# tkeskita/smoothMesh

Measured on AMD Instinct MI355X. Metric: mesh-points smoothed/sec/node (100 iters) + achieved HBM GB/s vs roofline, higher is better.
Workload: dtype f64

## Files before the change

smoothmesh_amd/csrc/kernels_boundary.hpp:

```cpp
#pragma once
#include "kernels.hpp"

namespace smgpu {

constexpr uint8_t BF_CORNER = 1, BF_FEATURE = 2, BF_SMOOTHSURF = 4, BF_CONNECTED = 8, BF_SHARP = 16;
constexpr int BND_ERR_NORMAL = 3, BND_ERR_NOHIT = 4, BND_ERR_STRING = 5;

struct BndView {
    int nB;
    const int* pts;
    uint8_t* flags;
    const double* corner;
    const int* inner;
    const int* bfOff; const int* bfVal;
    const uint8_t* ptClass;
    int nFeat;
    const int* featPts; const int* featString; const int* featOfBnd;
    double* featSum; int* featCnt;
    int nTE;
    const double* tePts; const int* teEdges; const int* teString;
    const int* strOff; const int* strEdges;
    int nNodes;
    const float* wideBox;
    const int* wideRef;
    const double* triVerts;
    double distanceTolerance, internalBlend;
};

__device__ __forceinline__ V3 faceAreaOf(const MeshView& m, const double* __restrict__ P, int f) {
    const int b = m.faceOff[f];
    const int n = m.faceOff[f + 1] - b;
    if (n == 3) {
        const V3 p0 = ldv(P, m.facePts[b]), p1 = ldv(P, m.facePts[b + 1]), p2 = ldv(P, m.facePts[b + 2]);
        return 0.5 * cross(p1 - p0, p2 - p0);
    }
    V3 fCentre = ldv(P, m.facePts[b]);
    for (int i = 1; i < n; ++i) fCentre = fCentre + ldv(P, m.facePts[b + i]);
    fCentre = fCentre / double(n);
    V3 sumN = v3(0, 0, 0);
    double sumA = 0.0;
    V3 thisPoint = ldv(P, m.facePts[b]);
    const V3 first = thisPoint;
    for (int i = 0; i < n; ++i) {
        const V3 nextPoint = (i == n - 1) ? first : ldv(P, m.facePts[b + i + 1]);
        const V3 nn = cross(nextPoint - thisPoint, fCentre - thisPoint);
        sumN = sumN + nn;
        sumA += mag(nn);
        thisPoint = nextPoint;
    }
    if (sumA < SMGPU_ROOTVSMALL) return v3(0, 0, 0);
    return 0.5 * sumN;
}

__device__ __forceinline__ void bndNormalsOf(const MeshView& m, const State& s, const BndView& b, int i) {
    if (s.acc->stop) return;
    if (i >= b.nB) return;
    const int p = b.pts[i];
    V3 n = ldv(s.layerNormal, p);
    const int f0 = b.bfOff[i], f1 = b.bfOff[i + 1];
    for (int k = f0; k < f1; ++k) {
        const V3 cSf = faceAreaOf(m, s.ptsCur, b.bfVal[k]);
        n = n - cSf / mag(cSf);
    }
    if (s.sharedSlot && s.sharedSlot[p] >= 0) { stv(s.layerNormal, p, n); return; }
    uint8_t fl = b.flags[i];
    if (f1 > f0) {
        if (mag(n) < 0.1) { n = v3(0, 0, 0); fl |= BF_SHARP; }
        else fl &= (uint8_t)~BF_SHARP;
        b.flags[i] = fl;
    }
    if (n != v3(0, 0, 0)) n = n / mag(n);
    stv(s.layerNormal, p, n);
}
__global__ void __launch_bounds__(kBlock) k_bnd_normals(MeshView m, State s, BndView b) { bndNormalsOf(m, s, b, blockIdx.x * kBlock + threadIdx.x); }

__device__ __forceinline__ void bndNormalsSharedOf(const State& s, const BndView& b, int nShared, const int* sharedLocal, int i) {
    if (s.acc->stop) return;
    if (i >= nShared) return;
    const int bi = s.bndOfShared[i];
    if (bi < 0) return;
    const double* r = s.combL + (size_t)i * s.lStride;
    V3 n = v3(r[0], r[1], r[2]);
    uint8_t fl = b.flags[bi];
    if (r[6] >= 1.0) {
        if (mag(n) < 0.1) { n = v3(0, 0, 0); fl |= BF_SHARP; }
        else fl &= (uint8_t)~BF_SHARP;
        b.flags[bi] = fl;
    }
    if (n != v3(0, 0, 0)) n = n / mag(n);
    stv(s.layerNormal, sharedLocal[i], n);
}
__global__ void __launch_bounds__(kBlock) k_bnd_normals_shared(State s, BndView b, int nShared, const int* sharedLocal) {
    bndNormalsSharedOf(s, b, nShared, sharedLocal, blockIdx.x * kBlock + threadIdx.x);
}
__global__ void __launch_bounds__(kBlock, 2) k_halo_combineAL(int nShared, const int* __restrict__ peer, const double* __restrict__ ownA,
                                                           const double* __restrict__ recvA, double* __restrict__ combA, int nBlocksTwo, int nMulti,
                                                           const int* multiIdx, const int* multiSlots, int nA, State s, BndView b, int bndOn,
                                                           const int* combOff, const int* combSlots, const double* ownL, const double* recvL,
                                                           double* combL, const int* sharedLocal, PushWait pw) {
    pushWait(pw);
    const int bx = (int)blockIdx.x;
    if (bx < nA) { haloCombineA2Of(bx, nShared, peer, ownA, recvA, combA, nBlocksTwo, nMulti, multiIdx, multiSlots, s.ownFold); return; }
    const int i = (bx - nA) * kBlock + (int)threadIdx.x;
    haloCombineLOf(i, nShared, combOff, combSlots, ownL, recvL, combL, s.lStride, s.ownFold);
    if (bndOn) bndNormalsSharedOf(s, b, nShared, sharedLocal, i);
}

__device__ __forceinline__ V3 projectToEdge(const BndView& b, const V3& pt, int e) {
    const V3 a = ldv(b.tePts, b.teEdges[2 * e]), c = ldv(b.tePts, b.teEdges[2 * e + 1]);
    const double edgeLength = mag(c - a);
    const V3 c2pt = pt - a, edgeVec = c - a;
    const double sN = dot(c2pt, edgeVec) / (edgeLength * edgeLength);
    if (sN <= 1e-6) return a;
    if (sN >= (1.0 - 1e-6)) return c;
    return a + sN * edgeVec;
}

__device__ __forceinline__ void bndFeatureOf(const MeshView& m, const State& s, const BndView& b, int j, int lane) {
    if (s.acc->stop) return;
    if (j >= b.nFeat) return;
    const int p = b.featPts[j], str = b.featString[j];
    V3 sum = v3(0, 0, 0);
    int cnt = 0;
    for (int k = m.ppOff[p]; k < m.ppOff[p + 1]; ++k) {
        const int q = m.ppPt[k];
        if (m.pflags[q] & PF_INTERNAL) continue;
        if (b.ptClass[q] & (BF_FEATURE | BF_CORNER)) continue;
        const V3 pt = ldv(s.ptsCur, q);
        double best = SMGPU_GREAT;
        int bestE = 0x7fffffff;
        V3 bestP = v3(SMGPU_GREAT, SMGPU_GREAT, SMGPU_GREAT);
        const int e0 = (str >= 0) ? b.strOff[str] : 0, e1 = (str >= 0) ? b.strOff[str + 1] : b.nTE;
        for (int ke = e0 + lane; ke < e1; ke += 64) {
            const int e = (str >= 0) ? b.strEdges[ke] : ke;
            const V3 pr = projectToEdge(b, pt, e);
            const double d = mag(pr - pt);
            if (d < best) { best = d; bestE = e; bestP = pr; }
        }
        for (int o = 32; o > 0; o >>= 1) {
            const double od = __shfl_xor(best, o, 64);
            const int oe = __shfl_xor(bestE, o, 64);
            const V3 op = v3(__shfl_xor(bestP.x, o, 64), __shfl_xor(bestP.y, o, 64), __shfl_xor(bestP.z, o, 64));
            if (od < best || (od == best && oe < bestE)) { best = od; bestE = oe; bestP = op; }
        }
        if (bestE == 0x7fffffff) { if (lane == 0) s.acc->err = BND_ERR_STRING; continue; }
        sum = sum + bestP;
        ++cnt;
    }
    if (lane == 0) { stv(b.featSum, j, sum); b.featCnt[j] = cnt; }
}
__global__ void __launch_bounds__(64) k_bnd_feature(MeshView m, State s, BndView b) { bndFeatureOf(m, s, b, (int)blockIdx.x, (int)threadIdx.x); }

template <int T, bool ORG>
__global__ void __launch_bounds__(T, (SMGPU_GEOM_WAVES * T) / 256) k_geom_tile_bnd(MeshView m, State s, GeomTileView g, int wantAvg, int writeFaces,
                                                  const int* tileList, int nLaunch, int xcdMap, int deferN, int deferIter, double* deferLocal,
                                                  double* deferHist, BndView b, int nBndBlocks, int nNormalBlocks) {
    const int bx = (int)blockIdx.x;
    if (bx < nBndBlocks) {
        if (bx < nNormalBlocks) bndNormalsOf(m, s, b, bx * T + (int)threadIdx.x);
        else bndFeatureOf(m, s, b, (bx - nNormalBlocks) * (T / 64) + ((int)threadIdx.x >> 6), (int)threadIdx.x & 63);
        return;
    }
    geomTileBody<T, ORG>(m, s, g, wantAvg, writeFaces, tileList, nLaunch, xcdMap, deferN, deferIter, deferLocal, deferHist, bx - nBndBlocks);
}

__device__ __forceinline__ bool triangleIntersection(const double* __restrict__ tv, const V3& orig, const V3& dir, double tol, double& t, V3& pt) {
    const V3 a = v3(tv[0], tv[1], tv[2]), bb = v3(tv[3], tv[4], tv[5]), c = v3(tv[6], tv[7], tv[8]);
    const V3 edge1 = bb - a, edge2 = c - a;
    const V3 pVec = cross(dir, edge2);
    const double det = dot(edge1, pVec);
    if (det > -SMGPU_ROOTVSMALL && det < SMGPU_ROOTVSMALL) return false;
    const double inv_det = 1.0 / det;
    const V3 tVec = orig - a;
    const double u = dot(tVec, pVec) * inv_det;
    if (u < -tol || u > 1.0 + tol) return false;
    const V3 qVec = cross(tVec, edge1);
    const double v = dot(dir, qVec) * inv_det;
    if (v < -tol || u + v > 1.0 + tol) return false;
    t = dot(edge2, qVec) * inv_det;
    if (t < -tol) return false;
    pt = a + u * edge1 + v * edge2;
    return true;
}

constexpr int kBvhStack = 64;

__device__ __forceinline__ bool findLine(const BndView& b, int* __restrict__ stack, const V3& start, const V3& end, V3& hitPoint) {
    const V3 dir = end - start;
    const double tol = 10.0 * 1.0e-15;
    const double o3[3] = {start.x, start.y, start.z}, d3[3] = {dir.x, dir.y, dir.z};
    double inv[3], oinv[3];
    bool flat[3], neg[3];
#pragma unroll
    for (int a = 0; a < 3; ++a) {
        flat[a] = d3[a] == 0.0;
        neg[a] = d3[a] < 0.0;
        inv[a] = flat[a] ? 0.0 : 1.0 / d3[a];
        oinv[a] = -(o3[a] * inv[a]);
    }
    double best = 0.0;
    int bestId = 0x7fffffff;
    double tLimit = 1.0 + 1e-6;
    int sp = 0;
    if (b.nNodes > 0) stack[kBlock * sp++] = 0;
    while (sp > 0) {
        const int item = stack[kBlock * --sp];
        if (item >= 0) {
            const float4* __restrict__ nb = reinterpret_cast<const float4*>(b.wideBox) + 12 * (size_t)item;
            float bx[48];
#pragma unroll
            for (int q = 0; q < 12; ++q) { const float4 v = nb[q]; bx[4 * q] = v.x; bx[4 * q + 1] = v.y; bx[4 * q + 2] = v.z; bx[4 * q + 3] = v.w; }
            const int4* __restrict__ rc = reinterpret_cast<const int4*>(b.wideRef) + 4 * (size_t)item;
            const int4 r0 = rc[0], r1 = rc[1], c0 = rc[2], c1 = rc[3];
            const int ref[8] = {r0.x, r0.y, r0.z, r0.w, r1.x, r1.y, r1.z, r1.w};
            const int cnt[8] = {c0.x, c0.y, c0.z, c0.w, c1.x, c1.y, c1.z, c1.w};
#pragma unroll
            for (int c = 0; c < 8; ++c) {
                const int n = cnt[c];
                double t0 = -1e-6, t1 = tLimit;
                bool touch = n >= 0;
#pragma unroll
                for (int a = 0; a < 3; ++a) {
                    const double lo = (double)bx[8 * a + c], hi = (double)bx[24 + 8 * a + c];
                    if (flat[a]) { touch = touch && !(o3[a] < lo || o3[a] > hi); }
                    else {
                        const double ta = fma(neg[a] ? hi : lo, inv[a], oinv[a]), tb = fma(neg[a] ? lo : hi, inv[a], oinv[a]);
                        t0 = (ta > t0) ? ta : t0;
                        t1 = (tb < t1) ? tb : t1;
                    }
                }
                if (touch && !(t0 > t1) && sp < kBvhStack) stack[kBlock * sp++] = (n == 0) ? ref[c] : -(16 * ref[c] + n) - 1;
            }
        } else {
            const int code = -(item + 1), first = code >> 4, n = code & 15;
            double tv[4][9];
            int ids[4];
#pragma unroll
            for (int k = 0; k < 4; ++k) {
                if (k < n) {
                    const double2* __restrict__ src = reinterpret_cast<const double2*>(b.triVerts) + 5 * (size_t)(first + k);
                    const double2 q0 = src[0], q1 = src[1], q2 = src[2], q3 = src[3], q4 = src[4];
                    tv[k][0] = q0.x; tv[k][1] = q0.y; tv[k][2] = q1.x; tv[k][3] = q1.y; tv[k][4] = q2.x; tv[k][5] = q2.y;
                    tv[k][6] = q3.x; tv[k][7] = q3.y; tv[k][8] = q4.x;
                    ids[k] = (int)__double_as_longlong(q4.y);
                }
            }
#pragma unroll
            for (int k = 0; k < 4; ++k) {
                double t;
                V3 pt;
                if (k >= n || !triangleIntersection(tv[k], start, dir, tol, t, pt)) continue;
                if (!(t <= 1.0)) continue;
                if (bestId == 0x7fffffff || t < best || (t == best && ids[k] < bestId)) { best = t; bestId = ids[k]; hitPoint = pt; }
            }
            if (bestId != 0x7fffffff) tLimit = fmin(tLimit, best + 1e-6 * (1.0 + fabs(best)));
        }
    }
    return bestId != 0x7fffffff;
}

__device__ __forceinline__ V3 findIntersectionPair(const BndView& b, int* __restrict__ stack, const V3& origPoint, const V3& pointNormal, double searchDistance, int role) {
    const V3 undef = v3(SMGPU_GREAT, SMGPU_GREAT, SMGPU_GREAT);
    const V3 endPoint1 = origPoint + pointNormal * searchDistance;
    const V3 endPoint2 = origPoint - pointNormal * searchDistance;
    V3 mine = undef, h;
    if (findLine(b, stack, origPoint, role ? endPoint2 : endPoint1, h)) mine = h;
    const V3 other = v3(__shfl_xor(mine.x, 1, 64), __shfl_xor(mine.y, 1, 64), __shfl_xor(mine.z, 1, 64));
    const V3 hitPoint1 = sel3(role, other, mine), hitPoint2 = sel3(role, mine, other);
    const double distance1 = mag(origPoint - hitPoint1);
    const double distance2 = mag(origPoint - hitPoint2);
    if (distance1 < distance2) return hitPoint1;
    else if (distance2 < distance1) return hitPoint2;
    if (findLine(b, stack, endPoint1, endPoint2, h)) return h;
    return undef;
}

template <bool FINAL>
__global__ void __launch_bounds__(kBlock) k_bnd_fix(MeshView m, State s, Prm prm, BndView b, int partialBase) {
    if (s.acc->stop) return;
    __shared__ int bvhStack[kBvhStack * kBlock];
    const int t = blockIdx.x * kBlock + threadIdx.x;
    const int i = t >> 1, role = t & 1;
    double dist = 0.0;
    int fcount = 0;
    if (i < b.nB) {
        const int p = b.pts[i];
        const uint8_t fl = b.flags[i];
        const V3 cur = ldv(s.ptsCur, p);
        V3 np = ldv(s.prop, p);
        const V3 undef = v3(SMGPU_GREAT, SMGPU_GREAT, SMGPU_GREAT);
        bool frozen = false;
        const int slot = s.sharedSlot ? s.sharedSlot[p] : -1;
        const double* cl = (slot >= 0) ? s.combL + (size_t)slot * s.lStride : nullptr;
        if (fl & BF_CORNER) np = ldv(b.corner, i);
        else if (fl & BF_FEATURE) {
            const int j = b.featOfBnd[i];
            if (cl) np = v3(cl[10], cl[11], cl[12]) / cl[13];
            else np = ldv(b.featSum, j) / double(b.featCnt[j]);
        } else if (fl & BF_SHARP) frozen = true;
        else if (fl & BF_SMOOTHSURF) {
            const V3 pointNormal = ldv(s.layerNormal, p);
            if (pointNormal == v3(0, 0, 0)) s.acc->err = BND_ERR_NORMAL;
            else {
                double searchDistance = b.distanceTolerance;
                V3 surfPoint = undef;
                for (int it = 0; it < 4; ++it) {
                    searchDistance *= (1.0 / 1e-4);
                    surfPoint = findIntersectionPair(b, bvhStack + threadIdx.x, np, pointNormal, searchDistance, role);
                    if (surfPoint != undef) { np = surfPoint; break; }
                }
                if (surfPoint == undef) s.acc->err = BND_ERR_NOHIT;
            }
        }
        if (role == 0) {
        if ((fl & BF_SMOOTHSURF) && (fl & BF_CONNECTED) && b.inner[i] >= 0 && !(fl & (BF_FEATURE | BF_CORNER | BF_SHARP))) {
            const V3 pointNormal = ldv(s.layerNormal, p);
// ... 52 lines not shown
```

smoothmesh_amd/csrc/kernels_tiled.hpp:

```cpp
#pragma once
#include "kernels.hpp"

#ifndef SMGPU_STAGGER
#define SMGPU_STAGGER 0
#endif
__device__ __forceinline__ void staggerFirstRound(int bid, int resident) {
#if SMGPU_STAGGER
    if (bid < resident) {
        const unsigned slot = __builtin_amdgcn_s_getreg((3 << 11) | (0 << 6) | 4) & 15u;
        for (unsigned k = 0; k < slot; ++k) __builtin_amdgcn_s_sleep(SMGPU_STAGGER);
    }
#else
    (void)bid; (void)resident;
#endif
}
#ifndef SMGPU_ABLATE
#define SMGPU_ABLATE 0
#endif
namespace smgpu {

constexpr unsigned kPad = 0xFFFFu;

struct GeomTileView {
    const int* cellOrder; const int* cellBeg; const int* tpOff; const int* tpIds; const int* tfOff; const int* tfIds;
    const int* fvBase; const uint8_t* fvWidth; const uint16_t* faceVerts;
    const int* cfBase; const uint8_t* cfWidth; const uint16_t* cellFaces;
    const uint8_t* tileFlags;
    const int* meta;
    int maxPoints, maxFaces;
};
struct GeomTileMeta { int tpOff, nPts, tfOff, nFaces, fvBase, fvWidth, cellBeg, nCells, cfBase, cfWidth, flags, pad; };
constexpr int kGeomMetaInts = 12;
typedef const __attribute__((address_space(4))) int* const_int_ptr;
__device__ __forceinline__ GeomTileMeta loadTileMeta(const GeomTileView& g, int tile) {
    const_int_ptr p = (const_int_ptr)(g.meta + (size_t)kGeomMetaInts * tile);
    GeomTileMeta t;
    t.tpOff = p[0]; t.nPts = p[1]; t.tfOff = p[2]; t.nFaces = p[3]; t.fvBase = p[4]; t.fvWidth = p[5];
    t.cellBeg = p[6]; t.nCells = p[7]; t.cfBase = p[8]; t.cfWidth = p[9]; t.flags = p[10]; t.pad = 0;
    return t;
}

struct SmoothTileView {
    const int* ptOrder; const int* ptBeg; const int* tcOff; const int* tcIds; const int* tnOff; const int* tnIds;
    const uint16_t* selfLoc;
    const int* pcBase; const uint8_t* pcWidth; const uint16_t* pcEll;
    const int* ppBase; const uint8_t* ppWidth; const uint16_t* ppEll;
    const uint16_t* pairEll;
    const int* pfBase; const uint8_t* pfWidth; const uint16_t* pfEll;
    const int* meta;
    int maxCells, maxPoints, usePairShare;
};

__device__ __forceinline__ SmoothTileView pickView(bool a, const SmoothTileView& x, const SmoothTileView& y) {
    SmoothTileView v;
#define SMGPU_PICK(F) v.F = a ? x.F : y.F;
    SMGPU_PICK(ptOrder) SMGPU_PICK(ptBeg) SMGPU_PICK(tcOff) SMGPU_PICK(tcIds) SMGPU_PICK(tnOff) SMGPU_PICK(tnIds) SMGPU_PICK(selfLoc)
    SMGPU_PICK(pcBase) SMGPU_PICK(pcWidth) SMGPU_PICK(pcEll) SMGPU_PICK(ppBase) SMGPU_PICK(ppWidth) SMGPU_PICK(ppEll) SMGPU_PICK(pairEll)
    SMGPU_PICK(pfBase) SMGPU_PICK(pfWidth) SMGPU_PICK(pfEll) SMGPU_PICK(meta) SMGPU_PICK(maxCells) SMGPU_PICK(maxPoints) SMGPU_PICK(usePairShare)
#undef SMGPU_PICK
    return v;
}

struct SmoothTileMeta { int ptBeg, nPts, tcOff, nCells, tnOff, nNbrs, pcBase, pcWidth, ppBase, ppWidth, pfBase, pfWidth; };
constexpr int kSmoothMetaInts = 12;
__device__ __forceinline__ SmoothTileMeta loadTileMeta(const SmoothTileView& g, int tile) {
    const_int_ptr p = (const_int_ptr)(g.meta + (size_t)kSmoothMetaInts * tile);
    SmoothTileMeta t;
    t.ptBeg = p[0]; t.nPts = p[1]; t.tcOff = p[2]; t.nCells = p[3]; t.tnOff = p[4]; t.nNbrs = p[5];
    t.pcBase = p[6]; t.pcWidth = p[7]; t.ppBase = p[8]; t.ppWidth = p[9]; t.pfBase = p[10]; t.pfWidth = p[11];
    return t;
}

__device__ __forceinline__ int launchTile(int n, int xcdMap, int b = (int)blockIdx.x) {
    if (!xcdMap) return b;
    const int per = (n + 7) >> 3;
    const int i = (b & 7) * per + (b >> 3);
    return i < n ? i : -1;
}
__host__ __device__ inline int tileGrid(int n, int xcdMap) { return xcdMap ? ((n + 7) >> 3) << 3 : n; }

__device__ __forceinline__ V3 ldsv(const double* x, const double* y, const double* z, int i) { return v3(x[i], y[i], z[i]); }

__device__ __forceinline__ void sqrtExact4(double m0, double m1, double m2, double m3, double& a0, double& a1, double& a2, double& a3) {
    const unsigned h0 = (unsigned)__double2hiint(m0), h1 = (unsigned)__double2hiint(m1), h2 = (unsigned)__double2hiint(m2),
                   h3 = (unsigned)__double2hiint(m3);
    const unsigned lo = min(min(h0, h1), min(h2, h3)), hi = max(max(h0, h1), max(h2, h3));
    if (SMGPU_FPEXACT_FAST && __builtin_expect(lo >= ((1023u - 767u) << 20) && hi < (2047u << 20), 1)) {
        a0 = sqrtCore(m0); a1 = sqrtCore(m1); a2 = sqrtCore(m2); a3 = sqrtCore(m3);
    } else {
        a0 = sqrt(m0); a1 = sqrt(m1); a2 = sqrt(m2); a3 = sqrt(m3);
    }
}

#define SMGPU_ELL_ENTRY(J, E, BODY) { const int j = (J); const unsigned e = (E); if (e != kPad) { BODY } }
#define SMGPU_ELL_FOREACH(ROWS, W4, STRIDE, BODY)                         \
    for (int c_ = 0; c_ < (W4); ++c_) {                                   \
        const ushort4 q_ = (ROWS)[(size_t)c_ * (STRIDE)];                 \
        SMGPU_ELL_ENTRY(4 * c_ + 0, q_.x, BODY)                           \
        SMGPU_ELL_ENTRY(4 * c_ + 1, q_.y, BODY)                           \
        SMGPU_ELL_ENTRY(4 * c_ + 2, q_.z, BODY)                           \
        SMGPU_ELL_ENTRY(4 * c_ + 3, q_.w, BODY)                           \
    }

#define SMGPU_ELL_CHUNK(C, Q, BODY)                                       \
    {                                                                     \
        SMGPU_ELL_ENTRY(4 * (C) + 0, (Q).x, BODY)                         \
        SMGPU_ELL_ENTRY(4 * (C) + 1, (Q).y, BODY)                         \
        SMGPU_ELL_ENTRY(4 * (C) + 2, (Q).z, BODY)                         \
        SMGPU_ELL_ENTRY(4 * (C) + 3, (Q).w, BODY)                         \
    }
#define SMGPU_ELL_FOREACH_PRE(Q0, Q1, ROWS, W4, STRIDE, BODY)             \
    {                                                                     \
        if ((W4) > 0) SMGPU_ELL_CHUNK(0, Q0, BODY)                        \
        if ((W4) > 1) SMGPU_ELL_CHUNK(1, Q1, BODY)                        \
        for (int c_ = 2; c_ < (W4); ++c_) {                               \
            const ushort4 q_ = (ROWS)[(size_t)c_ * (STRIDE)];             \
            SMGPU_ELL_CHUNK(c_, q_, BODY)                                 \
        }                                                                 \
    }

template <int T, int ROUNDS, int STRIDE = 1>
__device__ __forceinline__ void stageRecords(const double* __restrict__ src, const int* __restrict__ ids, int n, double* x,
                                             double* y, double* z, int tid) {
    for (int base = 0; base < n; base += T * ROUNDS) {
        int id[ROUNDS];
#pragma unroll
        for (int u = 0; u < ROUNDS; ++u) {
            const int i = base + u * T + tid;
            id[u] = (i < n) ? ids[i] : -1;
        }
        V3 v[ROUNDS];
#pragma unroll
        for (int u = 0; u < ROUNDS; ++u) v[u] = (id[u] >= 0) ? ldv(src, id[u]) : v3(0, 0, 0);
#pragma unroll
        for (int u = 0; u < ROUNDS; ++u) {
            const int i = base + u * T + tid;
            if (id[u] >= 0) { x[STRIDE * i] = v[u].x; y[STRIDE * i] = v[u].y; z[STRIDE * i] = v[u].z; }
        }
    }
}

template <int T, int R1, int R2>
__device__ __forceinline__ void stageRecords2(const double* __restrict__ s1, const int* __restrict__ i1, int n1, double* x1, double* y1,
                                              double* z1, const double* __restrict__ s2, const int* __restrict__ i2, int n2, double* x2,
                                              double* y2, double* z2, int tid) {
    if (n1 > T * R1 || n2 > T * R2) {
        stageRecords<T, R1>(s1, i1, n1, x1, y1, z1, tid);
        stageRecords<T, R2>(s2, i2, n2, x2, y2, z2, tid);
        return;
    }
    int a[R1], b[R2];
#pragma unroll
    for (int u = 0; u < R1; ++u) { const int i = u * T + tid; a[u] = (i < n1) ? i1[i] : -1; }
#pragma unroll
    for (int u = 0; u < R2; ++u) { const int i = u * T + tid; b[u] = (i < n2) ? i2[i] : -1; }
    V3 va[R1], vb[R2];
#pragma unroll
    for (int u = 0; u < R1; ++u) va[u] = (a[u] >= 0) ? ldv(s1, a[u]) : v3(0, 0, 0);
#pragma unroll
    for (int u = 0; u < R2; ++u) vb[u] = (b[u] >= 0) ? ldv(s2, b[u]) : v3(0, 0, 0);
#pragma unroll
    for (int u = 0; u < R1; ++u) { const int i = u * T + tid; if (a[u] >= 0) { x1[i] = va[u].x; y1[i] = va[u].y; z1[i] = va[u].z; } }
#pragma unroll
    for (int u = 0; u < R2; ++u) { const int i = u * T + tid; if (b[u] >= 0) { x2[i] = vb[u].x; y2[i] = vb[u].y; z2[i] = vb[u].z; } }
}

template <int T, int R>
__device__ __forceinline__ void stageRecordsPair(const double* __restrict__ s1, const double* __restrict__ s2, const int* __restrict__ ids,
                                                 int n, double* x1, double* y1, double* z1, double* x2, double* y2, double* z2, int tid) {
    for (int base = 0; base < n; base += T * R) {
        int id[R];
#pragma unroll
        for (int u = 0; u < R; ++u) { const int i = base + u * T + tid; id[u] = (i < n) ? ids[i] : -1; }
        V3 va[R], vb[R];
#pragma unroll
        for (int u = 0; u < R; ++u) { va[u] = (id[u] >= 0) ? ldv(s1, id[u]) : v3(0, 0, 0); vb[u] = (id[u] >= 0) ? ldv(s2, id[u]) : v3(0, 0, 0); }
#pragma unroll
        for (int u = 0; u < R; ++u) {
            const int i = base + u * T + tid;
            if (id[u] >= 0) { x1[i] = va[u].x; y1[i] = va[u].y; z1[i] = va[u].z; x2[i] = vb[u].x; y2[i] = vb[u].y; z2[i] = vb[u].z; }
        }
    }
}

template <int T>
__device__ __forceinline__ void stageRecordsCoh(const double* src, const int* __restrict__ ids, int n, double* x, double* y, double* z, int tid) {
    for (int i = tid; i < n; i += T) { const V3 v = ldvCoh(src, ids[i]); x[i] = v.x; y[i] = v.y; z[i] = v.z; }
}

#ifndef SMGPU_GEOM_AOS
#define SMGPU_GEOM_AOS 1
#endif
constexpr int kGP = SMGPU_GEOM_AOS ? 3 : 1;
#ifndef SMGPU_GEOM_LDS_B64
#define SMGPU_GEOM_LDS_B64 1
#endif
__device__ __forceinline__ V3 ldsg(const double* x, const double* y, const double* z, int i) {
#if SMGPU_GEOM_LDS_B64
    typedef const volatile __attribute__((address_space(3))) double* LdsPtr;
    const LdsPtr vx = (LdsPtr)x, vy = (LdsPtr)y, vz = (LdsPtr)z;
    return v3(vx[i], vy[i], vz[i]);
#else
    return v3(x[i], y[i], z[i]);
#endif
}
#ifndef SMGPU_GEOM_FACE_STRIDE
#define SMGPU_GEOM_FACE_STRIDE 6
#endif
constexpr int kGF = SMGPU_GEOM_AOS ? SMGPU_GEOM_FACE_STRIDE : 1;
struct GeomLds {
    double *px, *py, *pz;
    double *fcx, *fcy, *fcz;
    double *fax, *fay, *faz;
};
__device__ __forceinline__ GeomLds geomLds(double* lds, const GeomTileMeta& tm) {
    GeomLds L;
    if (SMGPU_GEOM_AOS) {
        L.px = lds;                      L.py = L.px + 1;  L.pz = L.px + 2;
        L.fcx = L.px + 3 * tm.nPts;      L.fcy = L.fcx + 1; L.fcz = L.fcx + 2;
        L.fax = L.fcx + 3;               L.fay = L.fcx + 4; L.faz = L.fcx + 5;
        return L;
    }
    L.px = lds;                  L.py = L.px + tm.nPts;    L.pz = L.py + tm.nPts;
    L.fcx = L.pz + tm.nPts;      L.fcy = L.fcx + tm.nFaces; L.fcz = L.fcy + tm.nFaces;
    L.fax = L.fcz + tm.nFaces;   L.fay = L.fax + tm.nFaces; L.faz = L.fay + tm.nFaces;
    return L;
}

template <bool ORG>
__device__ __forceinline__ void geomFace(const State& s, const GeomTileView& g, const GeomLds& L, const GeomTileMeta& tm, int i, unsigned tflags,
                                         int wantAvg, int writeFaces, bool pre = false, ushort4 preQ = make_ushort4(0, 0, 0, 0)) {
    const double *px = L.px, *py = L.py, *pz = L.pz;
    const int b = tm.tfOff;
    const int fw4 = tm.fvWidth >> 2;
    const ushort4* fvTile = reinterpret_cast<const ushort4*>(g.faceVerts + tm.fvBase);
    V3 fCentre, ctr, area;
    if (!ORG && (tflags & 1u)) {
        const ushort4 q = pre ? preQ : fvTile[i];
        const V3 p0 = ldsg(px, py, pz, kGP * (q.x)), p1 = ldsg(px, py, pz, kGP * (q.y)), p2 = ldsg(px, py, pz, kGP * (q.z)), p3 = ldsg(px, py, pz, kGP * (q.w));
        fCentre = divByCount(((p0 + p1) + p2) + p3, 4);
        V3 sumN = v3(0, 0, 0), sumAc = v3(0, 0, 0);
        double sumA = 0.0;
        const V3 n0 = cross(p1 - p0, fCentre - p0), n1 = cross(p2 - p1, fCentre - p1), n2 = cross(p3 - p2, fCentre - p2),
                 n3 = cross(p0 - p3, fCentre - p3);
        double a0, a1, a2, a3;
        sqrtExact4(magSqr(n0), magSqr(n1), magSqr(n2), magSqr(n3), a0, a1, a2, a3);
#define SMGPU_FAN4(THIS, NEXT, NN, A)                                          \
    {                                                                          \
        const V3 c = ((THIS) + (NEXT)) + fCentre;                              \
        sumN = sumN + (NN);                                                    \
        sumA += (A);                                                           \
        sumAc = sumAc + (A) * c;                                               \
    }
        SMGPU_FAN4(p0, p1, n0, a0) SMGPU_FAN4(p1, p2, n1, a1) SMGPU_FAN4(p2, p3, n2, a2) SMGPU_FAN4(p3, p0, n3, a3)
#undef SMGPU_FAN4
        if (sumA < SMGPU_ROOTVSMALL) { ctr = fCentre; area = v3(0, 0, 0); }
        else { ctr = divExact((1.0 / 3.0) * sumAc, sumA); area = 0.5 * sumN; }
    } else {
        const ushort4* row = fvTile + (size_t)i * fw4;
        fCentre = v3(0, 0, 0);
        int n = 0;
        SMGPU_ELL_FOREACH(row, fw4, 1, {
            const V3 p = ldsg(px, py, pz, kGP * (e));
            fCentre = (j == 0) ? p : fCentre + p;
            n = j + 1;
        })
        fCentre = divByCount(fCentre, n);
        if (n == 3) {
            const ushort4 q = row[0];
            const V3 p0 = ldsg(px, py, pz, kGP * (q.x)), p1 = ldsg(px, py, pz, kGP * (q.y)), p2 = ldsg(px, py, pz, kGP * (q.z));
            ctr = (1.0 / 3.0) * ((p0 + p1) + p2);
            area = 0.5 * cross(p1 - p0, p2 - p0);
        } else if (ORG) {
            V3 sumA = v3(0, 0, 0);
            V3 first = v3(0, 0, 0), thisPoint = v3(0, 0, 0);
            SMGPU_ELL_FOREACH(row, fw4, 1, {
                const V3 p = ldsg(px, py, pz, kGP * (e));
                if (j == 0) { first = p; thisPoint = p; }
                else { sumA = sumA + cross(p - thisPoint, fCentre - thisPoint); thisPoint = p; }
            })
            sumA = sumA + cross(first - thisPoint, fCentre - thisPoint);
            const V3 sumAHat = sumA / mag(sumA);
            double sumAn = 0.0;
            V3 sumAnc = v3(0, 0, 0);
#define SMGPU_FAN_ORG(NEXT)                                                    \
    {                                                                          \
        const V3 nextPoint = (NEXT);                                           \
        const V3 a = cross(nextPoint - thisPoint, fCentre - thisPoint);        \
        const V3 c = (thisPoint + nextPoint) + fCentre;                        \
        const double an = dot(a, sumAHat);                                     \
        sumAn += an;                                                           \
        sumAnc = sumAnc + an * c;                                              \
        thisPoint = nextPoint;                                                 \
    }
            SMGPU_ELL_FOREACH(row, fw4, 1, {
                const V3 p = ldsg(px, py, pz, kGP * (e));
                if (j == 0) { first = p; thisPoint = p; }
                else SMGPU_FAN_ORG(p)
            })
            SMGPU_FAN_ORG(first)
#undef SMGPU_FAN_ORG
            if (sumAn > SMGPU_VSMALL) ctr = ((1.0 / 3.0) * sumAnc) / sumAn;
            else ctr = fCentre;
            area = 0.5 * sumA;
        } else {
            V3 sumN = v3(0, 0, 0), sumAc = v3(0, 0, 0);
            double sumA = 0.0;
            V3 first = v3(0, 0, 0), thisPoint = v3(0, 0, 0);
#define SMGPU_FAN(NEXT)                                                        \
    {                                                                          \
        const V3 nextPoint = (NEXT);                                           \
        const V3 c = (thisPoint + nextPoint) + fCentre;                        \
        const V3 nn = cross(nextPoint - thisPoint, fCentre - thisPoint);       \
        const double a = sqrtExact(magSqr(nn));                                \
        sumN = sumN + nn;                                                      \
        sumA += a;                                                             \
        sumAc = sumAc + a * c;                                                 \
        thisPoint = nextPoint;                                                 \
    }
            SMGPU_ELL_FOREACH(row, fw4, 1, {
                const V3 p = ldsg(px, py, pz, kGP * (e));
                if (j == 0) { first = p; thisPoint = p; }
                else SMGPU_FAN(p)
            })
            SMGPU_FAN(first)
#undef SMGPU_FAN
            if (sumA < SMGPU_ROOTVSMALL) { ctr = fCentre; area = v3(0, 0, 0); }
            else { ctr = divExact((1.0 / 3.0) * sumAc, sumA); area = 0.5 * sumN; }
        }
    }
    L.fcx[kGF * i] = ctr.x; L.fcy[kGF * i] = ctr.y; L.fcz[kGF * i] = ctr.z;
    L.fax[kGF * i] = area.x; L.fay[kGF * i] = area.y; L.faz[kGF * i] = area.z;
    if (wantAvg && s.avgPacked) stv(s.fAvg, b + i, fCentre);
    if ((wantAvg && !s.avgPacked) || writeFaces) {
        const int fid = g.tfIds[b + i];
        if (fid < 0) {
            const int f = fid & 0x7fffffff;
            if (wantAvg && !s.avgPacked) stv(s.fAvg, f, fCentre);
            if (writeFaces) { stv(s.fCtr, f, ctr); stv(s.fArea, f, area); }
        }
    }
}

struct GeomCellIn { bool mine; int c; ushort4 qa, qb; };
template <int T>
__device__ __forceinline__ GeomCellIn geomCellLoad(const GeomTileView& g, const GeomTileMeta& tm, int tid, unsigned tflags) {
    GeomCellIn in;
    const int ci = tm.cellBeg + tid;
    in.mine = tid < tm.nCells;
    in.c = 0;
    in.qa = in.qb = make_ushort4(0, 0, 0, 0);
    if (in.mine) {
        in.c = g.cellOrder[ci];
        if ((tflags & 2u)) {
            const ushort4* row = reinterpret_cast<const ushort4*>(g.cellFaces + tm.cfBase) + tid;
            in.qa = row[0]; in.qb = row[T];
        }
    }
    return in;
}
template <int T, bool ORG>
__device__ __forceinline__ void geomCell(const State& s, const GeomTileView& g, const GeomLds& L, const GeomTileMeta& tm, int tid, unsigned tflags, const GeomCellIn& in,
                                         bool coh = false) {
    const double *fcx = L.fcx, *fcy = L.fcy, *fcz = L.fcz, *fax = L.fax, *fay = L.fay, *faz = L.faz;
    if (!in.mine) return;
    const int c = in.c;
    const int cw4 = tm.cfWidth >> 2;
    const ushort4* row = reinterpret_cast<const ushort4*>(g.cellFaces + tm.cfBase) + tid;
    V3 cEst = v3(0, 0, 0), ctr = v3(0, 0, 0);
    double vol = 0.0;
#define SMGPU_PYR(E, FC)                                                                                   \
    {                                                                                                      \
        const V3 fA = ldsg(fax, fay, faz, kGF * ((E) & 0x7fff));                                                   \
         \
        double pyr3Vol = dot(fA, (FC) - cEst);                                                             \
        pyr3Vol = ((E) & 0x8000) ? -pyr3Vol : pyr3Vol;                                                     \
        if (ORG) pyr3Vol = (pyr3Vol > SMGPU_VSMALL) ? pyr3Vol : SMGPU_VSMALL;    \
        const V3 pc = (3.0 / 4.0) * (FC) + (1.0 / 4.0) * cEst;                                             \
        ctr = ctr + pyr3Vol * pc;                                                                          \
        vol += pyr3Vol;                                                                                    \
    }
    if ((tflags & 2u)) {
        const ushort4 qa = in.qa, qb = in.qb;
        const unsigned e0 = qa.x, e1 = qa.y, e2 = qa.z, e3 = qa.w, e4 = qb.x, e5 = qb.y;
        const V3 c0 = ldsg(fcx, fcy, fcz, kGF * (e0 & 0x7fff)), c1 = ldsg(fcx, fcy, fcz, kGF * (e1 & 0x7fff)), c2 = ldsg(fcx, fcy, fcz, kGF * (e2 & 0x7fff)),
                 c3 = ldsg(fcx, fcy, fcz, kGF * (e3 & 0x7fff)), c4 = ldsg(fcx, fcy, fcz, kGF * (e4 & 0x7fff)), c5 = ldsg(fcx, fcy, fcz, kGF * (e5 & 0x7fff));
        cEst = cEst + c0; cEst = cEst + c1; cEst = cEst + c2; cEst = cEst + c3; cEst = cEst + c4; cEst = cEst + c5;
        cEst = divExact(cEst, 6.0);
        SMGPU_PYR(e0, c0) SMGPU_PYR(e1, c1) SMGPU_PYR(e2, c2) SMGPU_PYR(e3, c3) SMGPU_PYR(e4, c4) SMGPU_PYR(e5, c5)
    } else {
        int nFaces = 0;
        SMGPU_ELL_FOREACH(row, cw4, T, {
            cEst = cEst + ldsg(fcx, fcy, fcz, kGF * (e & 0x7fff));
            nFaces = j + 1;
        })
        cEst = divByCount(cEst, nFaces);
        SMGPU_ELL_FOREACH(row, cw4, T, {
            (void)j;
            const V3 fc = ldsg(fcx, fcy, fcz, kGF * (e & 0x7fff));
            SMGPU_PYR(e, fc)
        })
    }
#undef SMGPU_PYR
    if (fabs(vol) > SMGPU_VSMALL) ctr = divExact(ctr, vol);
    else ctr = cEst;
    if (coh) stvCoh(s.cellCtr, c, ctr); else stv(s.cellCtr, c, ctr);
}

#ifndef SMGPU_GEOM_WAVES
#define SMGPU_GEOM_WAVES 5
#endif
template <int T>
__device__ __forceinline__ void geomLoadIds(const GeomTileView& g, const GeomTileMeta& tm, int tid, int (&id)[2]) {
    const int* ids = g.tpIds + tm.tpOff;
#pragma unroll
    for (int u = 0; u < 2; ++u) { const int i = u * T + tid; id[u] = (i < tm.nPts) ? ids[i] : -1; }
}
struct GeomRows { ushort4 fq[2]; GeomCellIn cin; bool preFaces; };
template <int T, bool ORG>
__device__ __forceinline__ GeomRows geomLoadRows(const GeomTileView& g, const GeomTileMeta& tm, int tid) {
    GeomRows r;
    const unsigned tflags = (unsigned)tm.flags;
    r.preFaces = !ORG && (tflags & 1u);
#pragma unroll
    for (int u = 0; u < 2; ++u) {
        const int i = u * T + tid;
        r.fq[u] = (r.preFaces && i < tm.nFaces) ? reinterpret_cast<const ushort4*>(g.faceVerts + tm.fvBase)[i] : make_ushort4(0, 0, 0, 0);
    }
    r.cin = geomCellLoad<T>(g, tm, tid, tflags);
    return r;
}
__device__ __forceinline__ void geomLoadPoints(const State& s, const int (&id)[2], V3 (&v)[2]) {
#pragma unroll
    for (int u = 0; u < 2; ++u) v[u] = (id[u] >= 0) ? ldv(s.ptsCur, id[u]) : v3(0, 0, 0);
}
template <int T>
__device__ __forceinline__ void geomStorePoints(const State& s, const GeomTileView& g, const GeomTileMeta& tm, const GeomLds& L, const int (&id)[2],
                                                const V3 (&v)[2], int tid) {
#pragma unroll
    for (int u = 0; u < 2; ++u) {
        const int i = u * T + tid;
        if (id[u] >= 0) { L.px[kGP * i] = v[u].x; L.py[kGP * i] = v[u].y; L.pz[kGP * i] = v[u].z; }
    }
    if (tm.nPts > 2 * T)
        stageRecords<T, 2, kGP>(s.ptsCur, g.tpIds + tm.tpOff + 2 * T, tm.nPts - 2 * T, L.px + kGP * 2 * T, L.py + kGP * 2 * T, L.pz + kGP * 2 * T, tid);
}
template <int T, bool ORG>
__device__ __forceinline__ void geomFaces(const State& s, const GeomTileView& g, const GeomLds& L, const GeomTileMeta& tm, const GeomRows& r, int tid,
                                          int wantAvg, int writeFaces) {
    const unsigned tflags = (unsigned)tm.flags;
    const int nf = tm.nFaces;
#pragma unroll
    for (int u = 0; u < 2; ++u) {
        const int i = u * T + tid;
        if (i < nf) geomFace<ORG>(s, g, L, tm, i, tflags, wantAvg, writeFaces, r.preFaces, r.fq[u]);
    }
    for (int i = 2 * T + tid; i < nf; i += T) geomFace<ORG>(s, g, L, tm, i, tflags, wantAvg, writeFaces);
}

template <int T, bool ORG>
__device__ __forceinline__ void geomTileBody(const MeshView& m, const State& s, const GeomTileView& g, int wantAvg, int writeFaces, const int* tileList,
                                             int nLaunch, int xcdMap, int deferN, int deferIter, double* deferLocal, double* deferHist, int bid, bool coh = false) {
    const int stopped = s.acc->stop;
    const int li = launchTile(nLaunch, xcdMap, bid);
    if (li < 0) return;
    staggerFirstRound(bid, 256 * 4);
    if (deferN > 0 && bid == 0) { if (stopped) return; finishPartials<T>(s, deferN, deferIter, -1.0, deferLocal, deferHist); __syncthreads(); }
    extern __shared__ double lds[];
    const int tid = threadIdx.x;
    const int tile = tileList ? ((const_int_ptr)tileList)[li] : li;
    const GeomTileMeta tm = loadTileMeta(g, tile);
    const GeomLds L = geomLds(lds, tm);
    int id[2];
    geomLoadIds<T>(g, tm, tid, id);
    const GeomRows r = geomLoadRows<T, ORG>(g, tm, tid);
    V3 v[2];
    geomLoadPoints(s, id, v);
    geomStorePoints<T>(s, g, tm, L, id, v, tid);
    if (stopped) return;
    __syncthreads();
    if (SMGPU_ABLATE & 32) { if (tid < tm.nCells) stv(s.cellCtr, ((const_int_ptr)g.cellOrder)[tm.cellBeg + tid], v3(L.px[tid], 0.0, 0.0)); return; }
    geomFaces<T, ORG>(s, g, L, tm, r, tid, wantAvg, writeFaces);
    __syncthreads();
    if (SMGPU_ABLATE & 64) return;
    geomCell<T, ORG>(s, g, L, tm, tid, (unsigned)tm.flags, r.cin, coh);
}
template <int T, bool ORG>
__global__ void __launch_bounds__(T, (SMGPU_GEOM_WAVES * T) / 256) k_geom_tile(MeshView m, State s, GeomTileView g, int wantAvg, int writeFaces, const int* tileList,
                                                  int nLaunch, int xcdMap, int deferN, int deferIter, double* deferLocal,
                                                  double* deferHist) {
    geomTileBody<T, ORG>(m, s, g, wantAvg, writeFaces, tileList, nLaunch, xcdMap, deferN, deferIter, deferLocal, deferHist, (int)blockIdx.x);
}

struct SmoothLds { double *cx, *cy, *cz, *nx, *ny, *nz; };
__device__ __forceinline__ SmoothLds smoothLds(double* lds, const SmoothTileMeta& tm) {
    SmoothLds L;
    L.cx = lds;                 L.cy = L.cx + tm.nCells;  L.cz = L.cy + tm.nCells;
    L.nx = L.cz + tm.nCells;    L.ny = L.nx + tm.nNbrs;   L.nz = L.ny + tm.nNbrs;
    return L;
}
struct Top3 {
    double l1 = 0, l2 = 0, l3 = 0;
    unsigned w1 = 0xFFFFFFFFu, w2 = 0xFFFFFFFFu, w3 = 0xFFFFFFFFu;
    __device__ __forceinline__ void offer(double len, int j, unsigned e, bool take) {
        const unsigned w = ((unsigned)j << 16) | e;
        const bool b1 = take && (w1 == 0xFFFFFFFFu || len < l1);
        const bool b2 = take && !b1 && (w2 == 0xFFFFFFFFu || len < l2);
        const bool b3 = take && !b1 && !b2 && (w3 == 0xFFFFFFFFu || len < l3);
        const bool b12 = b1 || b2;
        l3 = b12 ? l2 : (b3 ? len : l3);  w3 = b12 ? w2 : (b3 ? w : w3);
        l2 = b1 ? l1 : (b2 ? len : l2);   w2 = b1 ? w1 : (b2 ? w : w2);
        l1 = b1 ? len : l1;               w1 = b1 ? w : w1;
    }
    __device__ __forceinline__ bool has2() const { return w2 != 0xFFFFFFFFu; }
    __device__ __forceinline__ bool has3() const { return w3 != 0xFFFFFFFFu; }
    __device__ __forceinline__ int k1() const { return (int)(w1 >> 16); }
    __device__ __forceinline__ int k2() const { return (int)(w2 >> 16); }
};
struct SmoothRow {
    bool mine; int p, selfL, wn4, wc4, slot;
    int peer, dst0, ndst;
    unsigned fl;
    const ushort4 *ppRow, *pcRow;
    ushort4 pp0, pp1, pc0, pc1;
    ushort4 pe0, pe1;
};
template <int T>
__device__ __forceinline__ unsigned pairBits(const SmoothTileView& g, const SmoothTileMeta& tm, const SmoothRow& R, int tid, int k) {
    if (k < 8) {
        const ushort4 q = (k & 4) ? R.pe1 : R.pe0;
        const unsigned lo = (k & 1) ? q.y : q.x, hi = (k & 1) ? q.w : q.z;
        return (k & 2) ? hi : lo;
    }
    const uint16_t* pe = g.pairEll + tm.ppBase;
    return pe[((size_t)(k >> 2) * T + tid) * 4 + (k & 3)];
}
struct SlotTabs { const int* slot; const int* peer; const int* dst0; const int* ndst; };
template <int T, bool COHC = false, int SLOTS = 1>
__device__ __forceinline__ SmoothRow smoothStage(const MeshView& m, const State& s, const SmoothTileView& g, const SmoothTileMeta& tm,
                                                 const SmoothLds& L, int tid, const SlotTabs& tb = SlotTabs{nullptr, nullptr, nullptr, nullptr}) {
    SmoothRow r;
    r.peer = -1; r.dst0 = -1; r.ndst = 0;
    r.mine = tid < tm.nPts;
    r.wn4 = tm.ppWidth >> 2; r.wc4 = tm.pcWidth >> 2;
    const int lane = r.mine ? tid : 0;
    r.ppRow = reinterpret_cast<const ushort4*>(g.ppEll + tm.ppBase) + tid;
    r.pcRow = reinterpret_cast<const ushort4*>(g.pcEll + tm.pcBase) + tid;
    const bool fast = tm.nCells <= 2 * T && tm.nNbrs <= 3 * T && r.wn4 > 0 && r.wc4 > 0;
    const ushort4 padq = make_ushort4(0xFFFF, 0xFFFF, 0xFFFF, 0xFFFF);
    if (fast) {
        const int* ic = g.tcIds + tm.tcOff;
        const int* in = g.tnIds + tm.tnOff;
        int a[2], b[3];
#pragma unroll
        for (int u = 0; u < 2; ++u) { const int i = u * T + tid; a[u] = (i < tm.nCells) ? ic[i] : -1; }
#pragma unroll
        for (int u = 0; u < 3; ++u) { const int i = u * T + tid; b[u] = (i < tm.nNbrs) ? in[i] : -1; }
        const int pi = tm.ptBeg + lane;
        const int p = g.ptOrder[pi];
        const int selfL = g.selfLoc[pi];
        const ushort4* ppl = reinterpret_cast<const ushort4*>(g.ppEll + tm.ppBase) + lane;
        const ushort4* pcl = reinterpret_cast<const ushort4*>(g.pcEll + tm.pcBase) + lane;
        const ushort4 pp0 = ppl[0], pp1 = ppl[r.wn4 > 1 ? T : 0], pc0 = pcl[0], pc1 = pcl[r.wc4 > 1 ? T : 0];
        const ushort4* pel = reinterpret_cast<const ushort4*>((g.usePairShare ? g.pairEll : g.ppEll) + tm.ppBase) + lane;
        r.pe0 = pel[0]; r.pe1 = pel[r.wn4 > 1 ? T : 0];
        int slot = -1, peer = -1, dst0 = -1, ndst = 0;
        if (SLOTS == 2) { slot = tb.slot[pi]; if (tb.peer) { peer = tb.peer[pi]; dst0 = tb.dst0[pi]; ndst = tb.ndst[pi]; } }
        V3 va[2], vb[3];
#pragma unroll
        for (int u = 0; u < 2; ++u) va[u] = (a[u] >= 0) ? (COHC ? ldvCoh(s.cellCtr, a[u]) : ldv(s.cellCtr, a[u])) : v3(0, 0, 0);
#pragma unroll
        for (int u = 0; u < 3; ++u) vb[u] = (b[u] >= 0) ? ldv(s.ptsCur, b[u]) : v3(0, 0, 0);
        const unsigned fl = m.pflags[p];
        if (SLOTS == 1) slot = s.sharedSlot ? s.sharedSlot[p] : -1;
#pragma unroll
        for (int u = 0; u < 2; ++u) { const int i = u * T + tid; if (a[u] >= 0) { L.cx[i] = va[u].x; L.cy[i] = va[u].y; L.cz[i] = va[u].z; } }
#pragma unroll
        for (int u = 0; u < 3; ++u) { const int i = u * T + tid; if (b[u] >= 0) { L.nx[i] = vb[u].x; L.ny[i] = vb[u].y; L.nz[i] = vb[u].z; } }
        r.p = r.mine ? p : 0; r.selfL = r.mine ? selfL : 0;
        r.fl = fl; r.slot = r.mine ? slot : -1; r.peer = r.mine ? peer : -1; r.dst0 = dst0; r.ndst = r.mine ? ndst : 0;
        r.pp0 = r.mine ? pp0 : padq; r.pp1 = (r.mine && r.wn4 > 1) ? pp1 : padq;
        r.pc0 = r.mine ? pc0 : padq; r.pc1 = (r.mine && r.wc4 > 1) ? pc1 : padq;
        return r;
    }
    r.p = 0; r.selfL = 0; r.fl = 0; r.slot = -1;
    r.pp0 = padq; r.pp1 = padq; r.pc0 = padq; r.pc1 = padq; r.pe0 = padq; r.pe1 = padq;
    if (r.mine) {
        if (g.usePairShare) {
            const ushort4* peRow = reinterpret_cast<const ushort4*>(g.pairEll + tm.ppBase) + tid;
            if (r.wn4 > 0) r.pe0 = peRow[0];
            if (r.wn4 > 1) r.pe1 = peRow[T];
        }
        const int pi = tm.ptBeg + tid;
        r.p = g.ptOrder[pi];
        r.selfL = g.selfLoc[pi];
        if (r.wn4 > 0) r.pp0 = r.ppRow[0];
        if (r.wn4 > 1) r.pp1 = r.ppRow[T];
        if (r.wc4 > 0) r.pc0 = r.pcRow[0];
        if (r.wc4 > 1) r.pc1 = r.pcRow[T];
        r.fl = m.pflags[r.p];
        if (SLOTS == 1) r.slot = s.sharedSlot ? s.sharedSlot[r.p] : -1;
        if (SLOTS == 2) { r.slot = tb.slot[pi]; if (tb.peer) { r.peer = tb.peer[pi]; r.dst0 = tb.dst0[pi]; r.ndst = tb.ndst[pi]; } }
    }
    if (COHC) stageRecordsCoh<T>(s.cellCtr, g.tcIds + tm.tcOff, tm.nCells, L.cx, L.cy, L.cz, tid);
    else stageRecords<T, 2>(s.cellCtr, g.tcIds + tm.tcOff, tm.nCells, L.cx, L.cy, L.cz, tid);
    stageRecords<T, 3>(s.ptsCur, g.tnIds + tm.tnOff, tm.nNbrs, L.nx, L.ny, L.nz, tid);
    return r;
}

template <bool FINAL, int T, int MODE = 0>
__device__ __forceinline__ void smoothPoint(const MeshView& m, const State& s, const Prm& prm, const SmoothTileView& g, const SmoothLds& L,
                                            const SmoothRow& R, const SmoothTileMeta& tm, int tid, double& dist, int& fcount, bool spTile = false) {
    const double *cx = L.cx, *cy = L.cy, *cz = L.cz, *nx = L.nx, *ny = L.ny, *nz = L.nz;
    const bool mine = R.mine;
    const int p = R.p, selfL = R.selfL, wn4 = R.wn4, wc4 = R.wc4;
    const ushort4 *ppRow = R.ppRow, *pcRow = R.pcRow;
    const ushort4 pp0 = R.pp0, pp1 = R.pp1, pc0 = R.pc0, pc1 = R.pc1;
    if ((SMGPU_ABLATE & 16) && !spTile) { if (mine) stv(FINAL ? s.ptsNext : s.prop, p, ldsv(nx, ny, nz, selfL)); return; }
    if (mine && !(MODE == 2 && !spTile && R.slot >= 0)) {
        const unsigned fl = R.fl;
        const bool internal = fl & PF_INTERNAL;
        const V3 cur = ldsv(nx, ny, nz, selfL);
        V3 sum = v3(0, 0, 0), r1, r2, r3;
        double m1 = 0.0, m2 = 0.0, m3 = 0.0;
        int count = 0, hc = 0;
        double shortestCur = SMGPU_GREAT;
        const int slot = (MODE == 1 || (MODE == 2 && !spTile)) ? -1 : R.slot;
        if (slot >= 0) {
            {
                const double* r = s.combA + (size_t)slot * SMGPU_HALO_A_DOUBLES;
                double w[SMGPU_HALO_A_DOUBLES];
#pragma unroll
                for (int q = 0; q < SMGPU_HALO_A_DOUBLES; ++q) w[q] = (MODE == 2 && R.peer < 0) ? ldCoh(r + q) : r[q];
                sum = v3(w[0], w[1], w[2]);
                r1 = v3(w[3], w[4], w[5]); r2 = v3(w[6], w[7], w[8]); r3 = v3(w[9], w[10], w[11]);
                const long long pk = __double_as_longlong(w[12]);
                count = (int)(pk & 0xffffffffll);
                hc = (int)(pk >> 32);
            }
            m1 = mag(r1); m2 = mag(r2); m3 = mag(r3);
            SMGPU_ELL_FOREACH_PRE(pp0, pp1, ppRow, wn4, T, {
                (void)j;
                const double len = mag(cur - ldsv(nx, ny, nz, e & 0x7fff));
                if (len < shortestCur) shortestCur = len;
            })
        } else {
            if (internal || prm.bndOn) {
                if (!(SMGPU_ABLATE & 8))
                SMGPU_ELL_FOREACH_PRE(pc0, pc1, pcRow, wc4, T, {
                    sum = sum + ldsv(cx, cy, cz, (SMGPU_ABLATE & 2) ? 0 : e);
                    count = j + 1;
                })
            }
            Top3 t3;
            SMGPU_ELL_FOREACH_PRE(pp0, pp1, ppRow, wn4, T, {
                const V3 dv_ = cur - ldsv(nx, ny, nz, (SMGPU_ABLATE & 2) ? 0 : (e & 0x7fff));
                const double len = (SMGPU_ABLATE & 1) ? magSqr(dv_) : mag(dv_);
                if (len < shortestCur) shortestCur = len;
                t3.offer(len, j, e, internal || !(e & 0x8000));
            })
            if (!t3.has2()) { s.acc->err = 1; r1 = r2 = r3 = v3(0, 0, 0); }
            else {
                r1 = ldsv(nx, ny, nz, t3.w1 & 0x7fff) - cur;
                r2 = ldsv(nx, ny, nz, t3.w2 & 0x7fff) - cur;
                r3 = !t3.has3() ? v3(SMGPU_GREAT, SMGPU_GREAT, SMGPU_GREAT) : ldsv(nx, ny, nz, t3.w3 & 0x7fff) - cur;
                m1 = t3.l1; m2 = t3.l2; m3 = !t3.has3() ? mag(r3) : t3.l3;
                if (g.usePairShare) {
                    hc = (pairBits<T>(g, tm, R, tid, t3.k1()) >> t3.k2()) & 1;
                } else {
                    const int nb = m.ppOff[p];
                    hc = shareCell(m, m.ppPt[nb + t3.k1()], m.ppPt[nb + t3.k2()]) ? 1 : 0;
                }
            }
        }
        V3 np = cur;
        if (count) np = divByCount(sum, count);
        const double blendFrac = arRatioLen(r1, r2, m1, m2, m3, hc != 0, internal);
        if (blendFrac > 0.0) {
            const V3 aCoords = cur + 0.5 * (r1 + r2);
            np = (1.0 - blendFrac) * np + blendFrac * aCoords;
        }
        {
            const V3 stepDir = np - cur;
            const double len = mag(stepDir);
            const double globalScale = (len > prm.maxStep) ? prm.maxStep / (len * prm.relStepFrac) : 1.0;
            np = cur + (prm.relStepFrac * globalScale) * stepDir;
        }
        if (prm.layersOn) np = layerTreat(s, prm, p, internal, cur, np);
        const bool deferBnd = prm.bndOn && !internal;
        if (prm.bndOn && internal) {
            const V3 stepDir = np - cur;
            const double len = mag(stepDir);
            const double globalScale = (len > prm.maxStep) ? prm.maxStep / (len * prm.relStepFrac) : 1.0;
            np = cur + (prm.relStepFrac * globalScale) * stepDir;
        }
        bool frozen = false;
        {
            double minSqr = __builtin_inf();
            if (!(SMGPU_ABLATE & 4))
            SMGPU_ELL_FOREACH_PRE(pp0, pp1, ppRow, wn4, T, {
                (void)j;
                const double t2 = magSqr(np - ldsv(nx, ny, nz, (SMGPU_ABLATE & 2) ? 0 : (e & 0x7fff)));
                if (t2 < minSqr) minSqr = t2;
            })
            const double rootMin = sqrtExact(minSqr);
            const double shortestNew = (rootMin < SMGPU_GREAT) ? rootMin : SMGPU_GREAT;
            const double shortest = (shortestNew < shortestCur) ? shortestNew : shortestCur;
            if (prm.totalMinFreeze && (shortest < prm.minEdge)) frozen = true;
            else if ((shortestNew < prm.minEdge) && (shortestNew < shortestCur)) frozen = true;
        }
        if (deferBnd) stv(s.prop, p, np);
        else if (FINAL && slot >= 0) {
            if (MODE == 2 && s.ownF) {
                stvCoh(s.prop, p, np);
                __hip_atomic_store(s.ownF + slot, frozen ? 1 : 0, __ATOMIC_RELAXED, __HIP_MEMORY_SCOPE_AGENT);
            } else stv(s.prop, p, np);
            s.frozen[p] = frozen ? 1 : 0;
            if (MODE == 2) {
                const int v = frozen ? 1 : 0;
                if (R.ndst == 1) { if (s.push.slotF) stPeer(s.push.slotF[R.dst0], v); else s.sendF[R.dst0] = v; }
                else
                    for (int k = s.sendOff[slot]; k < s.sendOff[slot + 1]; ++k) {
                        const int sl = s.sendSlots[k];
                        if (s.push.slotF) stPeer(s.push.slotF[sl], v); else s.sendF[sl] = v;
                    }
            } else if (s.inlinePackF)
                for (int k = s.sendOff[slot]; k < s.sendOff[slot + 1]; ++k) s.sendF[s.sendSlots[k]] = frozen ? 1 : 0;
        } else if (FINAL) {
            if (frozen || (!internal && !(fl & PF_SMOOTHSURF))) { np = cur; fcount = 1; }
            dist = mag(np - cur) / prm.maxStep;
            stv(s.ptsNext, p, np);
        } else {
            stv(s.prop, p, np);
            s.frozen[p] = frozen ? 1 : 0;
            if (s.stepSqr) s.stepSqr[p] = magSqr(np - cur);
        }
    }
}

template <bool FINAL, int T>
__global__ void __launch_bounds__(T) k_smooth_tile(MeshView m, State s, Prm prm, SmoothTileView g, const int* tileList,
                                                    int nLaunch, int xcdMap) {
    const int stopped = s.acc->stop;
    const int li = launchTile(nLaunch, xcdMap);
    if (li < 0) return;
    staggerFirstRound((int)blockIdx.x, 256 * 6);
    extern __shared__ double lds[];
    const int tile = tileList ? ((const_int_ptr)tileList)[li] : li, tid = threadIdx.x;
    const SmoothTileMeta tm = loadTileMeta(g, tile);
    const SmoothLds L = smoothLds(lds, tm);
    const SmoothRow R = smoothStage<T>(m, s, g, tm, L, tid);
    if (stopped) return;
    __syncthreads();
    double dist = 0.0;
    int fcount = 0;
    smoothPoint<FINAL, T>(m, s, prm, g, L, R, tm, tid, dist, fcount);
    if (FINAL) blockPublish<T>(s, dist, fcount, tile);
}

struct PackView {
    double* ownA; double* sendA;
    const int* sendOff; const int* sendSlots;
    int centroidAll;
};
template <int T, bool COHC = false, bool SP = false>
__device__ __forceinline__ void packTileBody(const MeshView& m, const State& s, const SmoothTileView& g, const PackView& pk, const int* tileList, int nLaunch,
                                             int xcdMap, int bid) {
    const int li = launchTile(nLaunch, xcdMap, bid);
    if (li < 0) return;
    extern __shared__ double lds[];
    const int tile = tileList ? ((const_int_ptr)tileList)[li] : li, tid = threadIdx.x;
    const SmoothTileMeta tm = loadTileMeta(g, tile);
    const SmoothLds L = smoothLds(lds, tm);
    const SmoothRow R = smoothStage<T, COHC, SP ? 2 : 1>(m, s, g, tm, L, tid, SlotTabs{s.spSlot, s.spPeer, s.spDst0, s.spNDst});
    __syncthreads();
    if (!R.mine) return;
    const int p = R.p;
    const int slot = R.slot;
    if (slot < 0) return;
    const double *cx = L.cx, *cy = L.cy, *cz = L.cz, *nx = L.nx, *ny = L.ny, *nz = L.nz;
    const int wn4 = R.wn4, wc4 = R.wc4;
    const ushort4 *ppRow = R.ppRow, *pcRow = R.pcRow;
    const ushort4 pp0 = R.pp0, pp1 = R.pp1, pc0 = R.pc0, pc1 = R.pc1;
    const bool internal = R.fl & PF_INTERNAL;
    const V3 cur = ldsv(nx, ny, nz, R.selfL);
    V3 sum = v3(0, 0, 0), r1, r2, r3;
    int count = 0, hc = 0;
    if (internal || pk.centroidAll) {
        SMGPU_ELL_FOREACH_PRE(pc0, pc1, pcRow, wc4, T, {
            sum = sum + ldsv(cx, cy, cz, e);
            count = j + 1;
        })
    }
    Top3 t3;
    SMGPU_ELL_FOREACH_PRE(pp0, pp1, ppRow, wn4, T, {
        const double len = mag(cur - ldsv(nx, ny, nz, e & 0x7fff));
        t3.offer(len, j, e, internal || !(e & 0x8000));
    })
    if (!t3.has2()) { s.acc->err = 1; r1 = r2 = r3 = v3(0, 0, 0); }
    else {
        r1 = ldsv(nx, ny, nz, t3.w1 & 0x7fff) - cur;
        r2 = ldsv(nx, ny, nz, t3.w2 & 0x7fff) - cur;
        r3 = !t3.has3() ? v3(SMGPU_GREAT, SMGPU_GREAT, SMGPU_GREAT) : ldsv(nx, ny, nz, t3.w3 & 0x7fff) - cur;
        if (g.usePairShare) {
            hc = (pairBits<T>(g, tm, R, tid, t3.k1()) >> t3.k2()) & 1;
        } else {
            const int nb = m.ppOff[p];
            hc = shareCell(m, m.ppPt[nb + t3.k1()], m.ppPt[nb + t3.k2()]) ? 1 : 0;
        }
    }
    double rec[SMGPU_HALO_A_DOUBLES];
    rec[0] = sum.x; rec[1] = sum.y; rec[2] = sum.z;
    rec[3] = r1.x; rec[4] = r1.y; rec[5] = r1.z;
    rec[6] = r2.x; rec[7] = r2.y; rec[8] = r2.z;
    rec[9] = r3.x; rec[10] = r3.y; rec[11] = r3.z;
    rec[12] = __longlong_as_double(((long long)hc << 32) | (long long)(unsigned int)count);
    double* o = pk.ownA + (size_t)slot * SMGPU_HALO_A_DOUBLES;
#pragma unroll
    for (int q = 0; q < SMGPU_HALO_A_DOUBLES; ++q) o[q] = rec[q];
    const int kBeg = (SP && R.ndst == 1) ? 0 : pk.sendOff[slot], kEnd = (SP && R.ndst == 1) ? 1 : pk.sendOff[slot + 1];
    for (int k = kBeg; k < kEnd; ++k) {
        const int sl = (SP && R.ndst == 1) ? R.dst0 : pk.sendSlots[k];
        if (s.push.slotA) {
            double* d = s.push.slotA[sl];
            if (((size_t)d & 8u) == 0) {
#pragma unroll
                for (int q = 0; q < 12; q += 2) stPeer2(d + q, rec[q], rec[q + 1]);
                stPeer(d + 12, rec[12]);
            } else {
                stPeer(d, rec[0]);
#pragma unroll
                for (int q = 1; q < 13; q += 2) stPeer2(d + q, rec[q], rec[q + 1]);
            }
            continue;
        }
        double* d = pk.sendA + (size_t)sl * SMGPU_HALO_A_DOUBLES;
#pragma unroll
        for (int q = 0; q < SMGPU_HALO_A_DOUBLES; ++q) d[q] = rec[q];
    }
}
template <int T>
__global__ void __launch_bounds__(T) k_pack_tile(MeshView m, State s, SmoothTileView g, PackView pk, const int* tileList, int nLaunch,
                                                  int xcdMap, PackLArgs la, int nLBlocks, unsigned tag) {
    if (s.acc->stop) return;
    if ((int)blockIdx.x < nLBlocks) haloPackLOf(s, la, (int)blockIdx.x * T + (int)threadIdx.x);
    else packTileBody<T>(m, s, g, pk, tileList, nLaunch, xcdMap, (int)blockIdx.x - nLBlocks);
    pushSignal(s.push, 0, tag);
}

struct HaloG {
    const int* geomS; int nGeomS; const int* geomI; int nGeomI;
    int nI1;
    int nPack;
    unsigned* ticket; unsigned serial;
    unsigned tagA;
    int debug;
};
template <int T, bool ORG>
__global__ void __launch_bounds__(T, (SMGPU_GEOM_WAVES * T) / 256) k_geom_halo(MeshView m, State s, GeomTileView g, int writeFaces, HaloG hg, int xcdMap, int deferN,
                                                                              int deferIter, double* deferLocal, double* deferHist, SmoothTileView sg, PackView pk) {
    const int bid = (int)blockIdx.x, gS = tileGrid(hg.nGeomS, xcdMap), g1 = tileGrid(hg.nI1, xcdMap), gP = tileGrid(hg.nPack, xcdMap);
    if (bid >= gS + g1 && bid < gS + g1 + gP) {
        if (s.acc->stop || (hg.debug & 1)) return;
        __builtin_amdgcn_s_setprio(3);
        if (!(hg.debug & 2)) roleWait(hg.ticket, hg.serial, &s.acc->err);
        packTileBody<T, true, true>(m, s, sg, pk, nullptr, hg.nPack, xcdMap, bid - gS - g1);
        pushSignal(s.push, 0, hg.tagA, (unsigned)gP);
        return;
    }
    const bool first = bid < gS, second = !first && bid < gS + g1;
    const int* list = first ? hg.geomS : (second ? hg.geomI : hg.geomI + hg.nI1);
    const int n = first ? hg.nGeomS : (second ? hg.nI1 : hg.nGeomI - hg.nI1);
    const int b = first ? bid : (second ? bid - gS : bid - gS - g1 - gP);
    geomTileBody<T, ORG>(m, s, g, 0, writeFaces, list, n, xcdMap, first ? deferN : 0, deferIter, deferLocal, deferHist, b, first);
    if (first) roleDone(hg.ticket, hg.serial, (unsigned)gS >> 3);
}

struct HaloFix {
    int nFix;
    int nShared; const int* sharedLocal; const int* combOff; const int* combSlots; const int* recvF; int partialBase;
    PushWait pwF;
    unsigned* ticket; unsigned serial;
    int sysLoads;
};
struct HaloS {
    int nTiles;
    int nA;
    int nSp;
    int gM, nMultiBlocks, nMulti;
    const int* multiIdx; const int* multiSlots; double* combA;
    unsigned* ticket; unsigned serial;
    PushWait pwA; unsigned tagF;
};
template <int T>
__device__ __forceinline__ void haloFixBody(const MeshView& m, const State& s, const Prm& prm, const HaloFix& hf, int blk) {
    roleWait(hf.ticket, hf.serial, &s.acc->err);
    pushWait(hf.pwF);
    const int i = blk * T + (int)threadIdx.x;
    double dist = 0.0;
    int fcount = 0;
    if (i < hf.nShared) {
        const int p = hf.sharedLocal[i];
        int frz = __hip_atomic_load(s.ownF + i, __ATOMIC_RELAXED, __HIP_MEMORY_SCOPE_AGENT);
        for (int k = hf.combOff[i]; k < hf.combOff[i + 1]; ++k) {
            const int sl = hf.combSlots[k];
            if (sl >= 0) frz |= hf.sysLoads ? ldSys(hf.recvF + sl) : hf.recvF[sl];
        }
        s.frozen[p] = frz ? 1 : 0;
        const uint8_t fl = m.pflags[p];
        const V3 cur = ldv(s.ptsCur, p);
        V3 np = ldvCoh(s.prop, p);
        if (frz || (!(fl & PF_INTERNAL) && !(fl & PF_SMOOTHSURF))) { np = cur; fcount = 1; }
        dist = mag(np - cur) / prm.maxStep;
        stv(s.ptsNext, p, np);
    }
    blockPublish<T>(s, dist, fcount, hf.partialBase + blk);
}
template <int T>
__global__ void __launch_bounds__(T) k_smooth_halo(MeshView m, State s, Prm prm, SmoothTileView g, SmoothTileView sg, HaloS hs, int xcdMap, HaloFix hf) {
    const int bid = (int)blockIdx.x, tid = threadIdx.x;
    if (bid < hs.gM) {
        if (bid >= hs.nMultiBlocks) return;
        __builtin_amdgcn_s_setprio(3);
        pushWait(hs.pwA);
        combineMulti<true>(bid, hs.nMulti, hs.multiIdx, hs.multiSlots, s.ownA, s.recvA, hs.combA, s.ownFold);
        roleDoneSmall(hs.ticket, hs.serial, (unsigned)hs.nMultiBlocks);
        return;
    }
    extern __shared__ double lds[];
    const int gSp = tileGrid(hs.nSp, xcdMap), gA = tileGrid(hs.nA, xcdMap);
    const bool spTile = bid < hs.gM + gSp;
    if (!spTile && bid >= hs.gM + gSp + gA && bid < hs.gM + gSp + gA + hf.nFix) {
        const int blk = bid - hs.gM - gSp - gA;
        __builtin_amdgcn_s_setprio(3);
        if (blk * T < hf.nShared) haloFixBody<T>(m, s, prm, hf, blk);
        return;
    }
    if (spTile) __builtin_amdgcn_s_setprio(3);
    const SmoothTileView v = pickView(spTile, sg, g);
    const bool batchA = bid < hs.gM + gSp + gA;
    int li = spTile ? launchTile(hs.nSp, xcdMap, bid - hs.gM)
                    : (batchA ? launchTile(hs.nA, xcdMap, bid - hs.gM - gSp) : launchTile(hs.nTiles - hs.nA, xcdMap, bid - hs.gM - gSp - gA - hf.nFix));
    if (li < 0 && !spTile) return;
    if (!spTile && !batchA) li += hs.nA;
    const int tile = li >= 0 ? li : 0;
    const SmoothTileMeta tm = loadTileMeta(v, tile);
    const SmoothLds L = smoothLds(lds, tm);
    if (spTile) {
        const int pi = tm.ptBeg + ((tid < tm.nPts) ? tid : 0);
        const int slot = (li >= 0 && tid < tm.nPts) ? s.spSlot[pi] : -1, peer = (slot >= 0) ? s.spPeer[pi] : -1;
        pushWait(hs.pwA);
        if (peer >= 0)
            combineTwoToMemory(s.ownA + (size_t)slot * SMGPU_HALO_A_DOUBLES, s.recvA + (size_t)(peer & 0x3fffffff) * SMGPU_HALO_A_DOUBLES,
                               (peer & 0x40000000) != 0, s.ownFold, hs.combA + (size_t)slot * SMGPU_HALO_A_DOUBLES);
    }
    const SlotTabs tb{spTile ? s.spSlot : s.posSlot, spTile ? s.spPeer : nullptr, s.spDst0, s.spNDst};
    const SmoothRow R = smoothStage<T, false, 2>(m, s, v, tm, L, tid, tb);
    if (spTile && hs.nMultiBlocks > 0) roleWait(hs.ticket, hs.serial, &s.acc->err);
    __syncthreads();
    double dist = 0.0;
    int fcount = 0;
    if (li >= 0) smoothPoint<true, T, 2>(m, s, prm, v, L, R, tm, tid, dist, fcount, spTile);
    if (spTile) {
        if (hf.nFix > 0) roleDone(hf.ticket, hf.serial, (unsigned)gSp >> 3);
        pushSignal(s.push, 1, hs.tagF, (unsigned)gSp);
    } else blockPublish<T>(s, dist, fcount, tile);
}

}
```

smoothmesh_amd/csrc/quality_loop.hpp:

```cpp
static int64_t qualityTraceNumber(const smgpu_handle* h) { return h->iterCount - h->qt.since; }
static int qualityTraceDue(const smgpu_handle* h, int n) {
    const int64_t at = qualityTraceNumber(h);
    return (int)((at + n) / h->qt.interval - at / h->qt.interval);
}
static int qualityTraceBegin(smgpu_handle* h, int nIters) {
    if (qualityEnsure(h)) return 1;
    const MeshView& m = h->mv;
    QualityTraceHost& t = h->qt;
    if (!t.block.live()) {
        const size_t nFB = (size_t)std::max(1, qualityGrid(m.nFaces)), nCB = (size_t)std::max(1, qualityGrid(m.nCells));
        const size_t nT = h->useTiles ? (size_t)std::max(1, h->gt.nTiles) : 1;
        if (t.block.alloc(&t.cellCtr, 3 * (size_t)std::max(1, m.nCells)) || t.block.alloc(&t.facePart, nFB) ||
            t.block.alloc(&t.cellPart, std::max(nCB, nT)) || t.block.alloc(&t.cellFold, (size_t)std::max(1, qualityGrid((int)nT))) ||
            t.block.alloc(&t.acc, 1))
            return t.block.failed("the quality trace");
        HIP_OK(hipMemsetAsync(t.acc, 0, sizeof(Accum), h->stream));
    }
    return t.slab.begin(h->stream, qualityTraceDue(h, nIters));
}
static int qualityTraceQueue(smgpu_handle* h, int64_t number, const smgpu_iter_stats* gate, smgpu_quality_trace_record* out) {
    const MeshView& m = h->mv;
    State ts = h->st;
    ts.cellCtr = h->qt.cellCtr;
    ts.acc = h->qt.acc;
    ts.stats = nullptr;
    const bool fused = h->qt.fusedWanted && h->useTiles && h->gt.nTiles > 0;
    const int nFB = qualityGrid(m.nFaces);
    int nCB = qualityGrid(m.nCells);
    const QCell* cPart = h->qt.cellPart;
    if (h->useTiles) {
        const int nT = h->gt.nTiles;
        if (nT > 0)
            withGeomTile(h, [&](auto tile, auto org) {
                constexpr int T = decltype(tile)::value;
                constexpr bool ORG = decltype(org)::value;
                if (fused) {
                    ensureDynLds(k_quality_geom_tile<T, ORG>, h->device, h->geomLds);
                    hipLaunchKernelGGL((k_quality_geom_tile<T, ORG>), dim3(tileGrid(nT, h->xcdMap)), dim3(T), (uint32_t)h->geomLds, h->stream, h->mv, ts, h->gv, nT,
                                       h->xcdMap, h->qt.thr, h->qt.cellPart, gate);
                } else {
                    ensureDynLds(k_geom_tile<T, ORG>, h->device, h->geomLds);
                    hipLaunchKernelGGL((k_geom_tile<T, ORG>), dim3(tileGrid(nT, h->xcdMap)), dim3(T), (uint32_t)h->geomLds, h->stream, h->mv, ts, h->gv, 0, 1,
                                       (const int*)nullptr, nT, h->xcdMap, 0, 0, (double*)nullptr, (double*)nullptr);
                }
            });
    } else {
        if (m.nFaces > 0) hipLaunchKernelGGL(k_face_geom, dim3(gridFor(m.nFaces)), dim3(kBlock), 0, h->stream, m, ts, 0, h->foamOrg ? 1 : 0);
        if (m.nCells > 0) hipLaunchKernelGGL(k_cell_centres, dim3(gridFor(m.nCells)), dim3(kBlock), 0, h->stream, m, ts, h->foamOrg ? 1 : 0);
    }
    if (nFB > 0)
        hipLaunchKernelGGL(k_quality_faces<false>, dim3(nFB), dim3(kQualityBlock), 0, h->stream, m, ts.ptsCur, ts.fCtr, ts.fArea, ts.cellCtr, h->q.own, h->q.nei,
                           QCoupling<false>{}, h->qt.thr, h->qt.facePart, (double*)nullptr, (double*)nullptr);
    if (fused) {
        nCB = qualityGrid(h->gt.nTiles);
        hipLaunchKernelGGL(k_quality_trace_fold, dim3(nCB), dim3(kQualityBlock), 0, h->stream, h->qt.cellPart, h->gt.nTiles, h->qt.cellFold, gate);
        cPart = h->qt.cellFold;
    } else if (nCB > 0) {
        hipLaunchKernelGGL(k_quality_cells, dim3(nCB), dim3(kQualityBlock), 0, h->stream, m, ts.fCtr, ts.fArea, h->qt.thr, h->qt.cellPart, (double*)nullptr,
                           (double*)nullptr, (double*)nullptr);
    }
    hipLaunchKernelGGL(k_quality_trace_final, dim3(1), dim3(kQualityBlock), 0, h->stream, h->qt.facePart, nFB, cPart, nCB, m.nCells, m.nFaces, m.nInternalFaces,
                       (long long)number, out, gate);
    HIP_OK(hipGetLastError());
    return 0;
}

static int qualityGuardDisarm(smgpu_handle* h, bool release);
int smgpu_set_quality_trace(smgpu_handle* h, int32_t interval, const smgpu_quality_params* p) {
    if (!h) return fail("null handle");
    if (interval < 0) return fail("smgpu_set_quality_trace: interval < 0");
    if (h->haloOn) return fail(kQualityHaloRefusal);
    HIP_OK(hipSetDevice(h->device));
    if (qualityGuardDisarm(h, true)) return 1;
    h->qt.interval = interval;
    h->qt.since = h->iterCount;
    h->qt.slab.discard();
    h->qt.thr = qualityThresholds(p);
    if (interval == 0) {
        HIP_OK(hipStreamSynchronize(h->stream));
        h->qt.release();
    }
    return 0;
}
int smgpu_get_quality_trace(smgpu_handle* h, smgpu_quality_trace_record* out, int64_t cap, int64_t* n) {
    if (!h || !n) return fail("null argument");
    return h->qt.slab.drain(out, cap, n, "smgpu_get_quality_trace");
}

static int qualityGuardDisarm(smgpu_handle* h, bool release) {
    h->qg.armed = false;
    h->qg.tripPending = false;
    h->qg.state.armed = 0;
    if (release && h->qg.block.live()) {
        HIP_OK(hipStreamSynchronize(h->stream));
        h->qg.release();
    }
    return 0;
}
static int qualityGuardCopy(smgpu_handle* h, bool restore, int64_t number, bool needGood) {
    const long long n = 3 * (long long)h->mv.nPoints;
    const bool normals = h->layersOn && h->qg.normal && h->st.layerNormal;
    const double *s0 = restore ? h->qg.pts : h->st.ptsCur, *s1 = normals ? (restore ? h->qg.normal : h->st.layerNormal) : nullptr;
    double *d0 = restore ? h->st.ptsCur : h->qg.pts, *d1 = normals ? (restore ? h->st.layerNormal : h->qg.normal) : nullptr;
    const int grid = (int)std::max<long long>(1, ((n >> 1) + (long long)kGuardBlock * kGuardPer - 1) / ((long long)kGuardBlock * kGuardPer));
    if (normals) hipLaunchKernelGGL(k_quality_guard_snapshot<true>, dim3(grid), dim3(kGuardBlock), 0, h->stream, s0, d0, s1, d1, n, (long long)number, h->qg.dev, needGood ? 1 : 0);
    else hipLaunchKernelGGL(k_quality_guard_snapshot<false>, dim3(grid), dim3(kGuardBlock), 0, h->stream, s0, d0, s1, d1, n, (long long)number, h->qg.dev, needGood ? 1 : 0);
    HIP_OK(hipGetLastError());
    if (restore) { h->q.epoch++; h->geomAheadDone = false; }
    return 0;
}
static int qualityGuardQueue(smgpu_handle* h, const smgpu_quality_trace_record* rec, int64_t number, const smgpu_iter_stats* gate) {
    hipLaunchKernelGGL(k_quality_guard_verdict, dim3(1), dim3(64), 0, h->stream, rec, h->qg.dev, (unsigned)h->qg.prm.criteria, &h->st.acc->stop, gate);
    HIP_OK(hipGetLastError());
    return qualityGuardCopy(h, false, number, true);
}
static int qualityGuardAfterTrip(smgpu_handle* h) {
    h->qg.tripPending = false;
    if (qualityGuardCopy(h, true, -1, false)) return 1;
    int64_t good = h->qg.state.snapshotIteration;
    const int interval = h->qt.interval;
    int rc = 0;
    if (h->qg.prm.refine && interval > 1) {
        Uncounted scope(h);
        unsigned long long nearSaved[3] = {0, 0, 0};
        if (h->st.nearTotal) HIP_OK(hipMemcpyAsync(nearSaved, h->st.nearTotal, sizeof(nearSaved), hipMemcpyDeviceToHost, h->stream));
        HIP_OK(hipMemsetAsync(&h->qg.dev->tripped, 0, sizeof(int), h->stream));
        HIP_OK(hipStreamSynchronize(h->stream));
        h->qg.refining = true;
        h->qt.interval = 1;
        for (int step = 1; step < interval && !rc; ++step) {
            h->iterCount = h->qt.since + good;
            int32_t done = 0;
            rc = iterateBody(h, 1, 0.0, nullptr, &done);
            if (rc) break;
            if (done != 1 || h->qg.lastVerdict != kGuardGood) {
                rc = qualityGuardCopy(h, true, -1, false);
                break;
            }
            ++good;
        }
        h->qt.interval = interval;
        h->qg.refining = false;
        if (!rc && h->st.nearTotal) HIP_OK(hipMemcpyAsync(h->st.nearTotal, nearSaved, sizeof(nearSaved), hipMemcpyHostToDevice, h->stream));
        HIP_OK(hipStreamSynchronize(h->stream));
        if (rc) return 1;
    }
    h->qg.state.snapshotIteration = good;
    h->qg.state.restoredIteration = good;
    h->iterCount = h->qt.since + good;
    return qualityGuardDisarm(h, false);
}

int smgpu_set_quality_guard(smgpu_handle* h, const smgpu_quality_guard_params* p, int32_t on) {
    if (!h) return fail("null handle");
    HIP_OK(hipSetDevice(h->device));
    if (!on) return qualityGuardDisarm(h, true);
    const smgpu_quality_guard_params prm = p ? *p : smgpu_quality_guard_params{SMGPU_GUARD_NONPOSITIVE_VOLUME | SMGPU_GUARD_WRONG_ORIENTED, 1};
    const uint32_t all = SMGPU_GUARD_NONPOSITIVE_VOLUME | SMGPU_GUARD_WRONG_ORIENTED | SMGPU_GUARD_ERROR_NONORTH;
    if (prm.criteria == 0 || (prm.criteria & ~all)) return fail("smgpu_set_quality_guard: criteria must be a non-empty combination of SMGPU_GUARD_NONPOSITIVE_VOLUME, _WRONG_ORIENTED and _ERROR_NONORTH");
    if (h->haloOn) return fail(kQualityHaloRefusal);
    if (h->bndOn)
        return fail("smgpu_set_quality_guard: not available on an engine with boundary point smoothing (its point normals are a running blend across the "
                    "iterations and its corner lists are host state, neither of which the guard's snapshot holds)");
    if (h->qt.interval <= 0) return fail("smgpu_set_quality_guard: the guard judges the records of the quality trace; switch it on first (smgpu_set_quality_trace)");
    if (h->iterOpen) return fail("smgpu_set_quality_guard: between smgpu_iter_begin and smgpu_iter_end");
    if (qualityGuardDisarm(h, true)) return 1;
    if (flushDeferred(h)) return 1;
    if (qualityTraceBegin(h, 0)) return 1;
    QualityGuardHost& g = h->qg;
    const size_t n = 3 * (size_t)std::max(1, h->mv.nPoints);
    if (g.block.alloc(&g.dev, 1) || g.block.alloc(&g.rec, 1) || g.block.alloc(&g.pts, n) ||
        (h->layersOn && h->st.layerNormal && g.block.alloc(&g.normal, n)))
        return g.block.failed("the quality guard");
    HIP_OK(hipMemsetAsync(h->qg.dev, 0, sizeof(GuardDev), h->stream));
    HIP_OK(hipMemsetAsync(h->qg.rec, 0, sizeof(smgpu_quality_trace_record), h->stream));
    if (qualityTraceQueue(h, 0, nullptr, h->qg.rec)) { h->qg.release(); return 1; }
    HIP_OK(hipMemcpyAsync(&h->qg.dev->baseline, h->qg.rec, sizeof(smgpu_quality_trace_record), hipMemcpyDeviceToDevice, h->stream));
    h->qg.prm = prm;
    h->qg.state = smgpu_quality_guard_state{};
    if (qualityGuardCopy(h, false, qualityTraceNumber(h), false)) { h->qg.release(); return 1; }
    HIP_OK(hipMemcpyAsync(&h->qg.state.baseline, h->qg.rec, sizeof(smgpu_quality_trace_record), hipMemcpyDeviceToHost, h->stream));
    if (checkDeviceError(h)) { h->qg.release(); return 1; }
    h->qg.state.armed = 1;
    h->qg.state.snapshotIteration = qualityTraceNumber(h);
    h->qg.armed = true;
    return 0;
}
int smgpu_get_quality_guard(smgpu_handle* h, smgpu_quality_guard_state* out) {
    if (!h || !out) return fail("null argument");
    *out = h->qg.state;
    return 0;
}
int smgpu_quality_guard_restore(smgpu_handle* h) {
    if (!h) return fail("null handle");
    if (!h->qg.armed) return fail("smgpu_quality_guard_restore: the quality guard is not armed (smgpu_set_quality_guard)");
    HIP_OK(hipSetDevice(h->device));
// ... 356 lines not shown
```

smoothmesh_amd/csrc/smgpu.hip:

```cpp
#include <hip/hip_runtime.h>
#include <hip/hip_ext.h>

#include <algorithm>
#include <chrono>
#include <future>
#include <memory>
#include <mutex>
#include <cstdio>
#include <cstring>
#include <string>
#include <type_traits>
#include <vector>

#include "kernels.hpp"
#include "layers.hpp"
#include "kernels_tiled.hpp"
#include "kernels_walk.hpp"
#include "kernels_filter.hpp"
#include "kernels_boundary.hpp"
#include "kernels_quality.hpp"
#include "kernels_quality_geom.hpp"
#include "kernels_quality_motion.hpp"
#include "kernels_quality_trace.hpp"
#include "kernels_quality_guard.hpp"
// ... 1030 lines not shown
    if (!h || !o) return fail("null argument");
    const Topology& t = h->topo;
    o->nPoints = t.nPoints; o->nCells = t.nCells; o->nFaces = t.nFaces; o->nInternalFaces = t.nInternalFaces; o->nEdges = t.nEdges;
    o->nnzFacePoints = t.facePoints.nnz(); o->nnzPointCells = t.pointCells.nnz(); o->nnzPointPoints = (int64_t)t.pointPoints.size();
    o->nnzPointFaces = t.facePoints.nnz(); o->nnzEdgeFaces = t.edgeFaces.nnz(); o->nnzEdgeCells = t.edgeCells.nnz();
    o->nnzCellFaces = t.cellFacesGeom.nnz();
    o->deviceBytes = h->deviceBytes;
    return 0;
}

int smgpu_mesh_stats(smgpu_handle* h, double* minEdge, double* maxEdge) {
    if (!h) return fail("null handle");
    HIP_OK(hipSetDevice(h->device));
    unsigned long long* d = nullptr;
    HIP_OK(hipMalloc((void**)&d, 16));
    struct Release { void* p; ~Release() { if (p) (void)hipFree(p); } } release{d};
    const double big = 1.0e300, zero = 0.0;
    unsigned long long init[2];
    std::memcpy(&init[0], &big, 8);
    std::memcpy(&init[1], &zero, 8);
    HIP_OK(hipMemcpyAsync(d, init, 16, hipMemcpyHostToDevice, h->stream));
    hipLaunchKernelGGL(k_edge_stats, dim3(std::max(1, std::min(gridFor(h->mv.nEdges), 1024))), dim3(kBlock), 0, h->stream, h->mv, h->st.ptsCur, d, d + 1);
    unsigned long long out[2];
    HIP_OK(hipMemcpyAsync(out, d, 16, hipMemcpyDeviceToHost, h->stream));
    HIP_OK(hipStreamSynchronize(h->stream));
    std::memcpy(minEdge, &out[0], 8);
    std::memcpy(maxEdge, &out[1], 8);
    return 0;
}

namespace smgpu {
__device__ __forceinline__ uint64_t mix64(uint64_t z) {
    z += 0x9E3779B97F4A7C15ull; z = (z ^ (z >> 30)) * 0xBF58476D1CE4E5B9ull; z = (z ^ (z >> 27)) * 0x94D049BB133111EBull;
    return z ^ (z >> 31);
}
__device__ __forceinline__ double selftestArg(uint64_t seed, long i, int j) {
    const uint64_t r = mix64(seed + 8ull * (uint64_t)i + (uint64_t)j);
    const uint64_t mant = r & 0xFFFFFFFFFFFFFull, sign = r >> 63;
    const unsigned pick = (unsigned)((r >> 52) & 0x7ff);
    uint64_t expo;
    switch ((i + (j == 3 ? 0 : 0)) & 7) {
        case 0: case 1: case 2: expo = 1023 - 40 + pick % 80; break;
        case 3: return __longlong_as_double((long long)r);
        case 4: {
            const unsigned k = pick % 6;
            if (k == 0) return sign ? -0.0 : 0.0;
            if (k == 1) return __longlong_as_double((long long)((sign << 63) | mant));
            if (k == 2) return __longlong_as_double((long long)((sign << 63) | (0x7ffull << 52)));
            if (k == 3) return __longlong_as_double((long long)((0x7ffull << 52) | mant | 1));
            expo = 1 + pick % 60; break;
        }
        case 5: {
            const unsigned edges[6] = {1023 - 767, 1023 - 250, 1023 + 250, 2046, 1, 1023 - 969};
            expo = edges[pick % 6] + (pick / 6) % 5 - 2;
            if ((long long)expo < 1) expo = 1;
            if (expo > 2046) expo = 2046;
            break;
        }
        case 6: expo = 1 + pick % 2046; break;
        default: expo = 1023 - 300 + pick % 600; break;
    }
    const uint64_t sgn = (j == 0 && (i & 8)) ? 0 : sign;
    return __longlong_as_double((long long)((sgn << 63) | (expo << 52) | mant));
}
__device__ __forceinline__ bool sameBits(double a, double b) { return (a != a && b != b) || __double_as_longlong(a) == __double_as_longlong(b); }
__global__ void k_selftest_fpexact(uint64_t seed, long n, unsigned long long* bad) {
    unsigned long long mine = 0;
    for (long i = blockIdx.x * (long)blockDim.x + threadIdx.x; i < n; i += (long)gridDim.x * blockDim.x) {
        const double x = selftestArg(seed, i, 0), y = selftestArg(seed, i, 1), z = selftestArg(seed, i, 2), w = selftestArg(seed, i, 3);
        if (!sameBits(sqrtExact(x), sqrt(x))) ++mine;
        double a0, a1, a2, a3;
        sqrtExact4(fabs(x), fabs(y), z, fabs(w), a0, a1, a2, a3);
        if (!sameBits(a0, sqrt(fabs(x))) || !sameBits(a1, sqrt(fabs(y))) || !sameBits(a2, sqrt(z)) || !sameBits(a3, sqrt(fabs(w)))) ++mine;
        const V3 q = divExact(v3(x, y, z), w);
        if (!sameBits(q.x, x / w) || !sameBits(q.y, y / w) || !sameBits(q.z, z / w)) ++mine;
        const V3 q6 = divExact(v3(x, y, z), 6.0);
        if (!sameBits(q6.x, x / 6.0) || !sameBits(q6.y, y / 6.0) || !sameBits(q6.z, z / 6.0)) ++mine;
    }
    if (mine) atomicAdd(bad, mine);
}
}

int smgpu_debug_selftest_fpexact(int32_t device, uint64_t seed, int64_t n, int64_t* mismatches) {
    if (!mismatches || n < 0) return fail("smgpu_debug_selftest_fpexact: bad arguments");
    if (hipSetDevice(device) != hipSuccess) return fail("smgpu_debug_selftest_fpexact: hipSetDevice failed");
    unsigned long long* d = nullptr;
    if (hipMalloc(&d, sizeof(*d)) != hipSuccess) return fail("smgpu_debug_selftest_fpexact: hipMalloc failed");
    unsigned long long host = 0;
    bool ok = hipMemset(d, 0, sizeof(*d)) == hipSuccess;
    if (ok) {
        hipLaunchKernelGGL(smgpu::k_selftest_fpexact, dim3(2048), dim3(256), 0, 0, seed, (long)n, d);
        ok = hipGetLastError() == hipSuccess && hipMemcpy(&host, d, sizeof(host), hipMemcpyDeviceToHost) == hipSuccess;
    }
    (void)hipFree(d);
    if (!ok) return fail("smgpu_debug_selftest_fpexact: launch failed");
    *mismatches = (int64_t)host;
    return 0;
}

int smgpu_set_foam_variant(smgpu_handle* h, int32_t variant) {
    if (!h) return fail("null handle");
    if (variant != SMGPU_FOAM_COM && variant != SMGPU_FOAM_ORG) return fail("smgpu_set_foam_variant: unknown variant");
    h->foamOrg = variant == SMGPU_FOAM_ORG;
    h->q.epoch++;
    h->geomAheadDone = false;
    return 0;
}

int smgpu_set_sync_variant(smgpu_handle* h, int32_t variant) {
    if (!h) return fail("null handle");
    if (variant != SMGPU_SYNC_MASTER && variant != SMGPU_SYNC_OWN) return fail("smgpu_set_sync_variant: unknown variant");
    h->st.ownFold = variant == SMGPU_SYNC_OWN ? 1 : 0;
    return 0;
}

int smgpu_set_params(smgpu_handle* h, const smgpu_params* p) {
    if (!h || !p) return fail("null argument");
    if (!(p->maxStepLength > 0.0)) return fail("maxStepLength must be > 0");
    h->prm = *p;
    h->prmSet = true;
    h->walkMode = -1;
    h->walkSwitches = 0;
    h->walkDecisions = 0;
    if (h->nActiveHost) *(volatile int*)h->nActiveHost = -1;
    h->geomAheadDone = false;
    computeAlgoBytes(h);
    return 0;
}

extern "C++" {
template <typename K>
static void ensureDynLds(K kernel, int device, size_t bytes) {
    static std::mutex mu;
    static size_t have[64] = {0};
    if (bytes <= 64 * 1024 || device < 0 || device >= 64) return;
    std::lock_guard<std::mutex> lock(mu);
    if (have[device] >= bytes) return;
    if (hipFuncSetAttribute((const void*)kernel, hipFuncAttributeMaxDynamicSharedMemorySize, (int)bytes) == hipSuccess) have[device] = bytes;
    else (void)hipGetLastError();
}
template <class F>
static void withGeomTile(const smgpu_handle* h, F&& f) {
    auto variant = [&](auto t) {
        if (h->foamOrg) f(t, std::true_type{});
        else f(t, std::false_type{});
    };
    if (h->geomT == 64) variant(std::integral_constant<int, 64>{});
    else if (h->geomT == 128) variant(std::integral_constant<int, 128>{});
    else variant(std::integral_constant<int, 256>{});
}
template <bool FINAL, int T>
static void launchSmoothTile(smgpu_handle* h, const MeshView& m, const State& s, const Prm& prm, const int* tileList, int nTiles, hipEvent_t evA, hipEvent_t evB) {
    ensureDynLds(k_smooth_tile<FINAL, T>, h->device, h->smoothLds);
    hipExtLaunchKernelGGL((k_smooth_tile<FINAL, T>), dim3(tileGrid(nTiles, h->xcdMap)), dim3(T), (uint32_t)h->smoothLds, h->stream, evA, evB, 0, m, s, prm, h->sv,
                          tileList, nTiles, h->xcdMap);
}
template <bool FINAL>
static int launchBndFix(smgpu_handle* h, int partialBase) {
    if (h->bv.nB == 0) return 0;
    return launchK(h, K_BND, [&] {
        hipLaunchKernelGGL(k_bnd_fix<FINAL>, dim3(gridFor(2 * (int64_t)h->bv.nB)), dim3(kBlock), 0, h->stream, h->mv, h->st, makePrm(h), h->bv, partialBase);
    });
}
static int launchBndPre(smgpu_handle* h, const MeshView& m, const State& s, hipStream_t stream) {
    if (h->bv.nB == 0) return 0;
    return launchK(h, K_BND, [&] {
        hipLaunchKernelGGL(k_bnd_normals, dim3(gridFor(h->bv.nB)), dim3(kBlock), 0, stream, m, s, h->bv);
        if (h->bv.nFeat) hipLaunchKernelGGL(k_bnd_feature, dim3(h->bv.nFeat), dim3(64), 0, stream, m, s, h->bv);
    }, stream);
}
static int runBndPre(smgpu_handle* h) {
    if (h->bndOn && h->bndInGeom && h->useTiles && h->bv.nB > 0) return 0;
    if (!h->bndOn || !h->bndSide || h->bndPreInFlight || h->timing) return 0;
    if (depSignal(h, DEP_BND_FORK, h->stream, h->evBndFork) || depWait(h, DEP_BND_FORK, h->bndSide, h->evBndFork)) return 1;
    if (launchBndPre(h, h->mv, h->st, h->bndSide)) return 1;
    if (depSignal(h, DEP_BND_JOIN, h->bndSide, h->evBndJoin)) return 1;
    h->bndPreInFlight = true;
    return 0;
}
template <bool FINAL>
static int runSmooth(smgpu_handle* h, const MeshView& m, const State& s, const Prm& prm, const int* tileList = nullptr, int nList = 0) {
    const int kid = FINAL ? K_SMOOTH_FINAL : K_SMOOTH_PROP;
    const bool withBnd = h->bndOn && !h->haloOn;
    if (withBnd) {
        if (h->bndPreDone) h->bndPreDone = false;
        else if (h->bndPreInFlight) {
            if (depWait(h, DEP_BND_JOIN, h->stream, h->evBndJoin)) return 1;
            h->bndPreInFlight = false;
        } else if (launchBndPre(h, m, s, h->stream)) return 1;
    }
    if (h->useTiles) {
        const int nT = tileList ? nList : h->stl.nTiles;
        if (nT == 0) return 0;
        if (launchKDispatch(h, kid, [&](hipEvent_t evA, hipEvent_t evB) {
                if (h->smoothT == 64) launchSmoothTile<FINAL, 64>(h, m, s, prm, tileList, nT, evA, evB);
                else if (h->smoothT == 128) launchSmoothTile<FINAL, 128>(h, m, s, prm, tileList, nT, evA, evB);
                else launchSmoothTile<FINAL, 256>(h, m, s, prm, tileList, nT, evA, evB);
            })) return 1;
    } else if (launchK(h, kid, [&] { hipLaunchKernelGGL(k_smooth<FINAL>, dim3(gridFor(m.nPoints)), dim3(kBlock), 0, h->stream, m, s, prm); })) return 1;
    if (withBnd) {
        const int base = h->useTiles ? h->stl.nTiles : gridFor(m.nPoints);
        return launchK(h, K_BND, [&] { hipLaunchKernelGGL(k_bnd_fix<FINAL>, dim3(gridFor(2 * (int64_t)h->bv.nB)), dim3(kBlock), 0, h->stream, m, s, prm, h->bv, base); });
    }
    return 0;
}

}

static int runGeometry(smgpu_handle* h, const int* tileList = nullptr, int nList = 0, bool fromNext = false, bool withBndPre = false) {
    const MeshView& m = h->mv;
    State s = h->st;
    if (fromNext) s.ptsCur = h->st.ptsNext;
    const int wantAvg = h->prm.faceAngleConstraint ? 1 : 0;
    if (h->useTiles) {
        const int nT = tileList ? nList : h->gt.nTiles;
        if (nT == 0) return 0;
        const bool bnd = withBndPre && h->bndOn && h->bndInGeom && !fromNext && h->bv.nB > 0 && !h->bndPreInFlight && !h->bndPreDone;
        if (bnd) h->bndPreDone = true;
        return launchKDispatch(h, K_GEOM_TILE, [&](hipEvent_t evA, hipEvent_t evB) {
            withGeomTile(h, [&](auto tile, auto org) {
                constexpr int T = decltype(tile)::value;
                constexpr bool ORG = decltype(org)::value;
                if (bnd) {
                    const int nNormal = (h->bv.nB + T - 1) / T, nFeat = (h->bv.nFeat + (T / 64) - 1) / (T / 64);
                    const int nBnd = ((nNormal + nFeat + 7) / 8) * 8;
                    ensureDynLds(k_geom_tile_bnd<T, ORG>, h->device, h->geomLds);
                    hipExtLaunchKernelGGL((k_geom_tile_bnd<T, ORG>), dim3(nBnd + tileGrid(nT, h->xcdMap)), dim3(T), (uint32_t)h->geomLds, h->stream, evA, evB, 0, m, s,
                                          h->gv, wantAvg, h->writeFaces ? 1 : 0, tileList, nT, h->xcdMap, h->deferN, h->deferIter, h->deferLocal, h->deferHist, h->bv,
                                          nBnd, nNormal);
                } else {
                    ensureDynLds(k_geom_tile<T, ORG>, h->device, h->geomLds);
                    hipExtLaunchKernelGGL((k_geom_tile<T, ORG>), dim3(tileGrid(nT, h->xcdMap)), dim3(T), (uint32_t)h->geomLds, h->stream, evA, evB, 0, m, s, h->gv,
                                          wantAvg, h->writeFaces ? 1 : 0, tileList, nT, h->xcdMap, h->deferN, h->deferIter, h->deferLocal, h->deferHist);
                }
            });
            h->deferN = 0;
            h->deferLocal = h->deferHist = nullptr;
        });
    }
    if (launchK(h, K_FACE_GEOM, [&] { hipLaunchKernelGGL(k_face_geom, dim3(gridFor(m.nFaces)), dim3(kBlock), 0, h->stream, m, s, wantAvg, h->foamOrg ? 1 : 0); })) return 1;
    if (launchK(h, K_CELL_CENTRES, [&] { hipLaunchKernelGGL(k_cell_centres, dim3(gridFor(m.nCells)), dim3(kBlock), 0, h->stream, m, s, h->foamOrg ? 1 : 0); })) return 1;
    return 0;
}

static int ensureWalkBuffers(smgpu_handle* h) {
    if (h->walkAlloc) return 0;
    const Topology& t = h->topo;
    if (envInt("SMGPU_WALK_MEMO_STATS", 0) && !SMGPU_WALK_MEMO) return fail("SMGPU_WALK_MEMO_STATS needs a build with -DSMGPU_WALK_MEMO=1 (make HIPFLAGS+=-DSMGPU_WALK_MEMO=1)");
    if (envInt("SMGPU_WALK_MEMO_STATS", 0) && !h->dWalkMemo) {
        if (devAlloc(h, &h->dWalkMemo, (size_t)t.nPoints + 2)) return 1;
        HIP_OK(zeroNow(h->dWalkMemo, 0, ((size_t)t.nPoints + 2) * sizeof(unsigned long long)));
    }
    const size_t P = t.nPoints, E = t.pointPoints.size();
    h->walkBlocks = gridFor(t.nPoints);
    WalkView& w = h->wv;
    int rc = 0;
    rc |= devAlloc(h, &w.activeSlot, P);
    rc |= devAlloc(h, &w.blkA, (size_t)h->walkBlocks + 1);
    rc |= devAlloc(h, &w.blkE, (size_t)h->walkBlocks + 1);
    rc |= devAlloc(h, &w.header, 4);
    rc |= devAlloc(h, &w.actIds, P);
    rc |= devAlloc(h, &w.actEntOff, P + 1);
    rc |= devAlloc(h, &w.actBits, P);
    rc |= devAlloc(h, &w.entOwner, E + P);
    rc |= devAlloc(h, &w.entNbr, E);
    rc |= devAlloc(h, &w.entSlot, E);
    rc |= devAlloc(h, &w.entBits, E);
    rc |= devAlloc(h, &w.relSlot, P);
    rc |= devAlloc(h, &w.header2, 4);
    rc |= devAlloc(h, &w.relBits, P);
    rc |= devAlloc(h, &w.hdrPos, P);
    rc |= devAlloc(h, &w.items, E + P);
    rc |= devAlloc(h, &h->dWalkOps, 64);
    if (rc) return 1;
    HIP_OK(zeroNow(h->dWalkOps, 0, 64 * sizeof(unsigned long long)));
    if (h->walkStar && h->walkPack && h->walkCache && !SMGPU_WALK_MEMO) {
        StarCache& c = h->starCache;
        c.capacity = std::max(1, envInt("SMGPU_WALK_CACHE_CAP", (int)std::max<size_t>(131072, P / 8)));
        void* pool = nullptr;
        while (hipMalloc(&pool, (size_t)c.capacity * sizeof(StarRec)) != hipSuccess) {
            (void)hipGetLastError();
            pool = nullptr;
            if (c.capacity <= 4096) break;
            c.capacity /= 4;
        }
        if (!pool) {
            if (envInt("SMGPU_VERBOSE", 0) >= 1) std::fprintf(stderr, "[smgpu] no device memory for the stars' records: every star is staged from the addressing\n");
            c = StarCache{nullptr, nullptr, nullptr, 0};
            h->walkAlloc = true;
            return 0;
        }
        h->allocs.push_back(pool);
        h->deviceBytes += (int64_t)((size_t)c.capacity * sizeof(StarRec));
        c.pool = (StarRec*)pool;
        if (devAlloc(h, &c.slot, P) || devAlloc(h, &c.count, 4)) return 1;
        HIP_OK(hipMemsetAsync(c.slot, 0xFF, P * sizeof(int), h->stream));
        HIP_OK(hipMemsetAsync(c.count, 0, 4 * sizeof(int), h->stream));
    }
    h->walkAlloc = true;
    return 0;
}

static int ensurePinned(smgpu_handle* h, size_t bytes) {
    if (h->pinnedBytes >= bytes) return 0;
    if (h->pinned) HIP_OK(hipHostFree(h->pinned));
    h->pinned = nullptr;
    h->pinnedBytes = 0;
    const size_t want = bytes + bytes / 2 + 4096;
    HIP_OK(hipHostMalloc(&h->pinned, want, hipHostMallocDefault));
    h->pinnedBytes = want;
    return 0;
}

static void drainWalk(const WalkItem* __restrict items, int N, uint8_t* __restrict frozen, int* __restrict stack, int* __restrict out,
                      int* spIO, size_t* nOutIO) {
    int sp = *spIO;
    size_t nOut = *nOutIO;
    while (sp) {
        int i = stack[--sp];
        const WalkItem hd = items[i];
        unsigned sel = 2;
        if (!frozen[hd.slot]) {
            if (hd.bits & 3u) { frozen[hd.slot] = 1; out[nOut++] = hd.id; }
            else if (hd.bits & 64u) sel = 1;
        }
        for (++i; i < N && !(items[i].bits & 0x80u); ++i) {
            const WalkItem e = items[i];
            if (frozen[e.slot] || !(e.bits & sel)) continue;
            out[nOut++] = e.id;
            if (e.bits & 32u) frozen[e.slot] = 1;
            if (e.bits & 16u) { stack[sp++] = e.hpos; __builtin_prefetch(&items[e.hpos]); }
        }
    }
    *spIO = sp;
    *nOutIO = nOut;
}

static void replayWalk(const WalkItem* __restrict items, int N, int nA, const uint8_t* __restrict relBits, std::vector<uint8_t>& frozenV,
                       std::vector<int>& stackV, std::vector<int>& outV) {
    frozenV.resize((size_t)nA + 2);
    stackV.resize((size_t)nA + 8);
    if (outV.size() < (size_t)2 * N + 8) outV.resize((size_t)2 * N + 8);
    uint8_t* __restrict frozen = frozenV.data();
    int* __restrict stack = stackV.data();
    int* __restrict out = outV.data();
    for (int a = 0; a < nA; ++a) frozen[a] = (relBits[a] >> 2) & 1;
    frozen[nA] = 0;
    frozen[nA + 1] = 1;
    size_t nOut = 0;
    int sp = 0;
    unsigned sel = 2;
    for (int i = 0; i < N; ++i) {
        const WalkItem it = items[i];
        const unsigned bits = it.bits;
        const unsigned isH = bits >> 7;
        if (__builtin_expect((isH * (unsigned)sp) != 0, 0)) {
            int spT = sp;
            size_t nT = nOut;
            drainWalk(items, N, frozen, stack, out, &spT, &nT);
            sp = spT;
            nOut = nT;
        }
        const unsigned nf = frozen[it.slot] ^ 1u;
        const unsigned act = nf & (0u - (unsigned)((bits & sel) != 0));
        out[nOut] = it.id;
        nOut += act;
        frozen[it.slot] |= (uint8_t)(act & (bits >> 5));
        stack[sp] = it.hpos;
        sp += (int)(act & (bits >> 4));
        const unsigned selH = 2u - (nf & (bits >> 6));
        sel ^= (sel ^ selH) & (0u - isH);
    }
    {
        int spT = sp;
        size_t nT = nOut;
        drainWalk(items, N, frozen, stack, out, &spT, &nT);
        nOut = nT;
    }
    outV.resize(nOut);
}

static int spinSync(hipStream_t stream) {
    for (;;) {
        const hipError_t e = hipStreamQuery(stream);
        if (e == hipSuccess) return 0;
        if (e != hipErrorNotReady) return fail(std::string("hipStreamQuery: ") + hipGetErrorString(e));
// ... 832 lines not shown
    const int w = h->st.lStride > 0 ? h->st.lStride : SMGPU_HALO_L_LAYERS;
    std::vector<void*> a((size_t)std::max(h->nSend, 1), nullptr), l(a.size(), nullptr), f(a.size(), nullptr), flags((size_t)std::max(h->pushPeers, 1), nullptr);
    int k = 0;
    for (int o = 0; o < h->pushPeers; ++o) {
        for (int j = 0; j < h->pushCount[(size_t)o]; ++j, ++k) {
            const size_t rs = (size_t)h->pushRemoteBase[(size_t)o] + (size_t)j;
            a[(size_t)k] = (double*)h->pushRecvA[(size_t)o] + rs * SMGPU_HALO_A_DOUBLES;
            l[(size_t)k] = h->pushRecvL[(size_t)o] ? (void*)((double*)h->pushRecvL[(size_t)o] + rs * (size_t)w) : nullptr;
            f[(size_t)k] = (int32_t*)h->pushRecvF[(size_t)o] + rs;
        }
        flags[(size_t)o] = (unsigned*)h->pushFlags[(size_t)o] + 2 * (size_t)h->pushMyIndex[(size_t)o];
    }
    if (k != h->nSend) return fail("smgpu_halo_set_push: the peers' slot counts do not add up to nSend");
    HIP_OK(hipMemcpy(h->dSlotA, a.data(), a.size() * sizeof(void*), hipMemcpyHostToDevice));
    HIP_OK(hipMemcpy(h->dSlotL, l.data(), l.size() * sizeof(void*), hipMemcpyHostToDevice));
    HIP_OK(hipMemcpy(h->dSlotF, f.data(), f.size() * sizeof(void*), hipMemcpyHostToDevice));
    HIP_OK(hipMemcpy(h->dPeerFlag, flags.data(), flags.size() * sizeof(void*), hipMemcpyHostToDevice));
    h->pushStride = w;
    return 0;
}

int smgpu_halo_set_push(smgpu_handle* h, const smgpu_push_desc* d) {
    if (!h || !h->haloOn) return fail("halo not configured");
    HIP_OK(hipSetDevice(h->device));
    HIP_OK(hipDeviceSynchronize());
    if (!d) {
        h->pushOn = false; h->st.push = PushView{};
        h->st.inlineCombine = 0;
        h->st.inlinePackF = (h->useTiles && envInt("SMGPU_HALO_INLINE_PACKF", 0)) ? 1 : 0;
        return 0;
    }
    if (d->nPeers < 0 || d->nPeers > 64) return fail("smgpu_halo_set_push: at most 64 peers");
    if (h->nShared && !(h->useTiles && h->nSharedTiles > 0 && h->packTiles)) return fail("smgpu_halo_set_push: needs the tiled pack kernel (SMGPU_TILES / SMGPU_PACK_TILES)");
    if (h->useExch) return fail("smgpu_halo_set_push: the exchange stream arrangement does not apply (nothing is enqueued by the host)");
    h->pushPeers = d->nPeers;
    h->pushCount.assign(d->peerCount, d->peerCount + d->nPeers);
    h->pushRemoteBase.assign(d->remoteBase, d->remoteBase + d->nPeers);
    h->pushMyIndex.assign(d->myIndexAtPeer, d->myIndexAtPeer + d->nPeers);
    h->pushRecvA.assign(d->peerRecvA, d->peerRecvA + d->nPeers);
    h->pushRecvL.assign(d->peerRecvL, d->peerRecvL + d->nPeers);
    h->pushRecvF.assign(d->peerRecvF, d->peerRecvF + d->nPeers);
    h->pushFlags.assign(d->peerFlags, d->peerFlags + d->nPeers);
    h->pushLocalFlags = d->localFlags;
    for (int o = 0; o < d->nPeers; ++o)
        if (!h->pushRecvA[(size_t)o] || !h->pushRecvF[(size_t)o] || !h->pushFlags[(size_t)o] || h->pushMyIndex[(size_t)o] < 0 || h->pushMyIndex[(size_t)o] >= 64)
            return fail("smgpu_halo_set_push: incomplete peer description");
    if (!h->dSlotA) {
        const size_t n = (size_t)std::max(h->nSend, 1);
        void **a = nullptr, **l = nullptr, **f = nullptr, **pf = nullptr;
        if (devAlloc(h, &a, n) || devAlloc(h, &l, n) || devAlloc(h, &f, n) || devAlloc(h, &pf, 64) || devAlloc(h, &h->dPushTicket, 2)) return 1;
        h->dSlotA = a; h->dSlotL = l; h->dSlotF = f; h->dPeerFlag = pf;
        HIP_OK(zeroNow(h->dPushTicket, 0, 2 * sizeof(unsigned)));
    }
    if (pushBuildTables(h)) return 1;
    PushView pv;
    pv.slotA = (double* const*)h->dSlotA; pv.slotL = (double* const*)h->dSlotL; pv.slotF = (int* const*)h->dSlotF;
    pv.ticket = h->dPushTicket; pv.peerFlag = (unsigned* const*)h->dPeerFlag; pv.localFlag = (const unsigned*)h->pushLocalFlags; pv.nPeers = d->nPeers;
    pv.fence = envInt("SMGPU_PUSH_FENCE", 0) ? 1 : 0;
    h->pushTimeoutTicks = (unsigned long long)std::max(1, envInt("SMGPU_PUSH_TIMEOUT_S", 60)) * 100000000ull;
    h->st.push = pv;
    h->st.inlineCombine = 0;
    h->st.inlinePackF = 0;
    h->pushOn = true;
    return 0;
}

int smgpu_push_alloc(int32_t device, size_t bytes, void** ptr, void* ipcHandle64) {
    if (!ptr || !ipcHandle64 || bytes == 0) return fail("smgpu_push_alloc: bad argument");
    static_assert(sizeof(hipIpcMemHandle_t) == 64, "hipIpcMemHandle_t is 64 bytes");
    HIP_OK(hipSetDevice(device));
    void* p = nullptr;
    HIP_OK(hipExtMallocWithFlags(&p, bytes, hipDeviceMallocUncached));
    HIP_OK(hipMemset(p, 0, bytes));
    HIP_OK(hipDeviceSynchronize());
    hipIpcMemHandle_t hd;
    const hipError_t e = hipIpcGetMemHandle(&hd, p);
    if (e != hipSuccess) { (void)hipFree(p); return fail(std::string("hipIpcGetMemHandle: ") + hipGetErrorString(e)); }
    std::memcpy(ipcHandle64, &hd, 64);
    *ptr = p;
    return 0;
}
int smgpu_push_open(int32_t device, const void* ipcHandle64, void** ptr) {
    if (!ptr || !ipcHandle64) return fail("smgpu_push_open: bad argument");
    HIP_OK(hipSetDevice(device));
    hipIpcMemHandle_t hd;
    std::memcpy(&hd, ipcHandle64, 64);
    HIP_OK(hipIpcOpenMemHandle(ptr, hd, hipIpcMemLazyEnablePeerAccess));
    return 0;
}
int smgpu_push_close(void* ptr) { if (ptr) HIP_OK(hipIpcCloseMemHandle(ptr)); return 0; }
int smgpu_push_free(void* ptr) { if (ptr) HIP_OK(hipFree(ptr)); return 0; }

static bool flagUsable(const smgpu_handle* h) {
    const char* v = std::getenv("ROCPROF_COUNTER_COLLECTION");
    return h->useExch && h->flagWanted && h->streamOps && !h->pushOn && h->deviceShare == 1 && !(v && std::atoi(v) != 0) && h->sendA && h->sendF;
}
static int ensureFlagView(smgpu_handle* h) {
    if (h->flagBuilt) return 0;
    const size_t n = (size_t)std::max(h->nSend, 1);
    if (!h->dFlagWords) {
        void **a = nullptr, **f = nullptr, **pf = nullptr;
        if (devAlloc(h, &h->dFlagWords, 64) || devAlloc(h, &a, n) || devAlloc(h, &f, n) || devAlloc(h, &pf, 1) || devAlloc(h, &h->dSelfTicket, 2)) return 1;
        h->dSelfSlotA = a; h->dSelfSlotF = f; h->dSelfPeerFlag = pf;
    }
    std::vector<void*> a(n, nullptr), f(n, nullptr);
    for (int k = 0; k < h->nSend; ++k) { a[(size_t)k] = h->sendA + (size_t)k * SMGPU_HALO_A_DOUBLES; f[(size_t)k] = h->sendF + k; }
    void* w = h->dFlagWords;
    HIP_OK(hipMemcpy(h->dSelfSlotA, a.data(), n * sizeof(void*), hipMemcpyHostToDevice));
    HIP_OK(hipMemcpy(h->dSelfSlotF, f.data(), n * sizeof(void*), hipMemcpyHostToDevice));
    HIP_OK(hipMemcpy(h->dSelfPeerFlag, &w, sizeof(void*), hipMemcpyHostToDevice));
    HIP_OK(zeroNow(h->dFlagWords, 0, 64 * sizeof(uint32_t)));
    HIP_OK(zeroNow(h->dSelfTicket, 0, 2 * sizeof(unsigned)));
    PushView pv{};
    pv.slotA = (double* const*)h->dSelfSlotA; pv.slotL = nullptr; pv.slotF = (int* const*)h->dSelfSlotF;
    pv.ticket = h->dSelfTicket; pv.peerFlag = (unsigned* const*)h->dSelfPeerFlag; pv.localFlag = (const unsigned*)(h->dFlagWords + 16); pv.nPeers = 1;
    pv.fence = 0;
    h->flagView = pv;
    h->flagBuilt = true;
    return 0;
}
static int flagRelay(smgpu_handle* h, int writeIdx, int waitIdx) {
    const unsigned tag = (unsigned)(h->haloIter + 1);
    const unsigned long long ticks = (unsigned long long)std::max(1, envInt("SMGPU_PUSH_TIMEOUT_S", 60)) * 100000000ull;
    hipLaunchKernelGGL(k_flag_relay, dim3(1), dim3(64), 0, h->exch, writeIdx >= 0 ? h->dFlagWords + writeIdx : nullptr, tag,
                       waitIdx >= 0 ? (const unsigned*)(h->dFlagWords + waitIdx) : nullptr, tag, &h->st.acc->err, ticks);
    HIP_OK(hipGetLastError());
    return 0;
}
static bool mergedOk(const smgpu_handle* h) {
    const bool fused = !h->prm.edgeAngleConstraint && !h->prm.faceAngleConstraint;
    return h->mergedWanted && fused && h->useTiles && h->geomT == 256 && h->smoothT == 256 && h->nShared > 0 && h->shr.nTiles > 0 && h->nGeomShared > 0 &&
           h->packTiles && h->dMultiIdx && h->dPeer && h->dPosSlot && h->dRoleTickets && !h->layersOn && !h->bndOn && (!h->useExch || flagUsable(h)) && !h->geomAheadDone &&
           !h->st.inlinePackF &&
           h->xcdMap != 0 &&
           !(h->pushOn && h->deviceShare > 1 && h->shr.nTiles > 256);
}
static bool flagged(const smgpu_handle* h) { return h->mergedIter && h->useExch; }
static int runMergedGeomPack(smgpu_handle* h) {
    const MeshView& m = h->mv;
    State s = h->st;
    if (flagged(h)) s.push = h->flagView;
    const int slots = 4 * 256;
    const int gS = tileGrid(h->nGeomShared, h->xcdMap);
    const int nI1 = std::min(h->nGeomInterior, std::max(0, envInt("SMGPU_HALO_PACK_AFTER", flagged(h) ? 0 : slots + slots / 2) - gS) & ~7);
    const int g1 = tileGrid(nI1, h->xcdMap), g2 = tileGrid(h->nGeomInterior - nI1, h->xcdMap), gP = tileGrid(h->shr.nTiles, h->xcdMap);
    HaloG hg;
    hg.geomS = h->dGeomShared; hg.nGeomS = h->nGeomShared; hg.geomI = h->dGeomInterior; hg.nGeomI = h->nGeomInterior; hg.nI1 = nI1;
    hg.nPack = h->shr.nTiles;
    hg.ticket = h->dRoleTickets; hg.serial = ++h->roleLaunches[0];
    hg.tagA = (unsigned)(h->haloIter + 1);
    hg.debug = envInt("SMGPU_HALO_DEBUG", 0);
    const PackView pk{h->dOwnA, h->sendA, h->dSendOff, h->dSendSlots, 0};
    const size_t lds = std::max(h->geomLds, h->haloLds);
    const int rc = launchKDispatch(h, K_GEOM_TILE, [&](hipEvent_t evA, hipEvent_t evB) {
        if (h->foamOrg)
            hipExtLaunchKernelGGL((k_geom_halo<256, true>), dim3(gS + g1 + gP + g2), dim3(256), (uint32_t)lds, h->stream, evA, evB, 0, m, s, h->gv, h->writeFaces ? 1 : 0, hg,
                                  h->xcdMap, h->deferN, h->deferIter, h->deferLocal, h->deferHist, h->hv, pk);
        else
            hipExtLaunchKernelGGL((k_geom_halo<256, false>), dim3(gS + g1 + gP + g2), dim3(256), (uint32_t)lds, h->stream, evA, evB, 0, m, s, h->gv, h->writeFaces ? 1 : 0, hg,
                                  h->xcdMap, h->deferN, h->deferIter, h->deferLocal, h->deferHist, h->hv, pk);
    });
    h->deferN = 0;
    h->deferLocal = h->deferHist = nullptr;
    return rc;
}
static int runMergedSmooth(smgpu_handle* h) {
    const Prm prm = makePrm(h);
    HaloS hs;
    hs.nTiles = h->stl.nTiles; hs.nSp = h->shr.nTiles;
    hs.nMulti = h->nMulti; hs.nMultiBlocks = h->nMulti ? gridFor((int64_t)h->nMulti * 16) : 0;
    hs.gM = ((hs.nMultiBlocks + 7) / 8) * 8;
    hs.multiIdx = h->dMultiIdx; hs.multiSlots = h->dMultiSlots; hs.combA = h->dCombA;
    hs.ticket = h->dRoleTickets + kRoleWords;
    hs.serial = hs.nMultiBlocks ? ++h->roleLaunches[1] : 0u;
    hs.pwA = pushWaitOf(h, 0); hs.tagF = (unsigned)(h->haloIter + 1);
    HaloFix hf{};
    h->fixInSmooth = envInt("SMGPU_HALO_FIX_INSIDE", h->pushOn ? 1 : 0) != 0 && (h->pushOn || flagged(h));
    hs.nA = h->stl.nTiles;
    if (h->fixInSmooth) {
        hs.nA = (int)((int64_t)h->stl.nTiles * std::min(100, std::max(0, envInt("SMGPU_HALO_FIX_AT", flagged(h) ? 85 : 55))) / 100) & ~7;
        hf.nFix = ((gridFor(h->nShared) + 7) / 8) * 8;
        hf.nShared = h->nShared; hf.sharedLocal = h->dSharedLocal; hf.combOff = h->dCombOff; hf.combSlots = h->dCombSlots; hf.recvF = h->recvF;
        hf.partialBase = h->stl.nTiles;
        hf.pwF = pushWaitOf(h, 1);
        hf.ticket = h->dRoleTickets + 2 * kRoleWords; hf.serial = ++h->roleLaunches[2];
        hf.sysLoads = flagged(h) ? 1 : 0;
    }
    const int grid = hs.gM + tileGrid(h->shr.nTiles, h->xcdMap) + tileGrid(hs.nA, h->xcdMap) + hf.nFix + tileGrid(h->stl.nTiles - hs.nA, h->xcdMap);
    const size_t lds = std::max(h->smoothLds, h->haloLds);
    State s = h->st;
    if (flagged(h)) s.push = h->flagView;
    s.ownF = h->fixInSmooth ? h->dOwnF : nullptr;
    return launchKDispatch(h, K_SMOOTH_FINAL, [&](hipEvent_t evA, hipEvent_t evB) {
        hipExtLaunchKernelGGL((k_smooth_halo<256>), dim3(grid), dim3(256), (uint32_t)lds, h->stream, evA, evB, 0, h->mv, s, prm, h->sv, h->hv, hs, h->xcdMap, hf);
    });
}

int smgpu_iter_begin(smgpu_handle* h) {
    if (!h || !h->haloOn) return fail("halo not configured");
    if (!h->prmSet) return fail("smgpu_set_params has not been called");
    if (h->tg.coupled && h->tg.k >= 0)
        return fail("smgpu_iter_begin: the coupled tangle constraint has not finished the passes of the last iteration (smgpu_tangle_pass_begin / _end)");
    h->q.epoch++;
    h->iterOpen = true;
    HIP_OK(hipSetDevice(h->device));
    if (h->pushOn && h->pushStride != (h->st.lStride > 0 ? h->st.lStride : SMGPU_HALO_L_LAYERS)) {
        HIP_OK(hipStreamSynchronize(h->stream));
        if (pushBuildTables(h)) return 1;
    }
    h->st.stepSqr = swapApplyHalo(h) ? h->dStepSqr : nullptr;
    h->mergedIter = mergedOk(h);
    if (h->mergedIter) {
        if (h->useExch && ensureFlagView(h)) return 1;
        if (runMergedGeomPack(h)) return 1;
        if (updateWalkMode(h)) return 1;
        if (h->useExch) return flagRelay(h, -1, 0);
        return exchAfterCompute(h);
    }
    if (runBndPre(h)) return 1;
    if (h->geomAheadDone) {
        if (runGeometry(h, h->dGeomShared, h->nGeomShared, false, true)) return 1;
        h->geomAheadDone = false;
    } else if (runGeometry(h, nullptr, 0, false, true)) return 1;
    if (flushDeferred(h)) return 1;
    if (updateWalkMode(h)) return 1;
    if (forkFaFilter(h)) return 1;
    State s = h->st;
    const MeshView& m = h->mv;
    if (h->bndOn) {
        if (h->bndPreDone) h->bndPreDone = false;
        else if (h->bndPreInFlight) {
            if (depWait(h, DEP_BND_JOIN, h->stream, h->evBndJoin)) return 1;
            h->bndPreInFlight = false;
        } else if (launchBndPre(h, m, s, h->stream)) return 1;
    }
    if (h->nShared)
        if (launchK(h, K_HALO, [&] {
                const bool withL = h->layersOn || h->bndOn;
                const unsigned tag = (unsigned)(h->haloIter + 1);
                const PackLArgs la{h->dSharedLocal, h->dOwnL, h->nShared, h->dSendOff, h->dSendSlots, h->sendL, h->bv.bfOff, h->bv.inner, h->bv.featOfBnd,
                                   h->bv.featSum, h->bv.featCnt};
                if (h->useTiles && h->nSharedTiles > 0 && h->packTiles) {
                    const PackView pk{h->dOwnA, h->sendA, h->dSendOff, h->dSendSlots, h->bndOn ? 1 : 0};
                    const int T = h->smoothT, nL = withL ? (((h->nShared + T - 1) / T + 7) / 8) * 8 : 0;
                    const dim3 grid(nL + tileGrid(h->nSharedTiles, h->xcdMap));
                    if (T == 64) hipLaunchKernelGGL(k_pack_tile<64>, grid, dim3(64), h->smoothLds, h->stream, m, s, h->sv, pk, h->dSharedTiles, h->nSharedTiles, h->xcdMap, la, nL, tag);
                    else if (T == 128) hipLaunchKernelGGL(k_pack_tile<128>, grid, dim3(128), h->smoothLds, h->stream, m, s, h->sv, pk, h->dSharedTiles, h->nSharedTiles, h->xcdMap, la, nL, tag);
                    else hipLaunchKernelGGL(k_pack_tile<256>, grid, dim3(256), h->smoothLds, h->stream, m, s, h->sv, pk, h->dSharedTiles, h->nSharedTiles, h->xcdMap, la, nL, tag);
                } else {
                    hipLaunchKernelGGL(k_halo_packA, dim3(gridFor(h->nShared)), dim3(kBlock), 0, h->stream, m, s, h->dSharedLocal, h->dOwnA, h->nShared,
                                       h->dSendOff, h->dSendSlots, h->sendA, h->bndOn ? 1 : 0);
                    if (withL) hipLaunchKernelGGL(k_halo_packL, dim3(gridFor(h->nShared)), dim3(kBlock), 0, h->stream, s, la);
                }
            })) return 1;
    return exchAfterCompute(h);
}

int smgpu_iter_interior(smgpu_handle* h) {
    if (!h || !h->haloOn) return fail("halo not configured");
    HIP_OK(hipSetDevice(h->device));
    if (!h->useTiles || h->interiorDone || !h->useExch || h->mergedIter) return 0;
    const bool fused = !h->prm.edgeAngleConstraint && !h->prm.faceAngleConstraint;
    const Prm prm = makePrm(h);
    if (fused) { if (runSmooth<true>(h, h->mv, h->st, prm, h->dInteriorTiles, h->nInteriorTiles)) return 1; }
    else if (runSmooth<false>(h, h->mv, h->st, prm, h->dInteriorTiles, h->nInteriorTiles)) return 1;
    h->interiorDone = true;
    return 0;
}

int smgpu_iter_mid(smgpu_handle* h) {
    if (!h || !h->haloOn) return fail("halo not configured");
    HIP_OK(hipSetDevice(h->device));
    const bool fused = !h->prm.edgeAngleConstraint && !h->prm.faceAngleConstraint;
    const Prm prm = makePrm(h);
    if (h->mergedIter) {
        if (h->useExch) {
            if (runMergedSmooth(h)) return 1;
            return flagRelay(h, 16, 1);
        }
        if (runMergedSmooth(h)) return 1;
        return exchAfterCompute(h);
    }
    if (h->useTiles && !h->interiorDone && smgpu_iter_interior(h)) return 1;
    if (computeAfterExch(h)) return 1;
    if (h->nShared)
        if (launchK(h, K_HALO, [&] {
                const int nTwo = h->st.inlineCombine ? 0 : gridFor(h->nShared), nMultiBlocks = h->nMulti ? gridFor((int64_t)h->nMulti * 16) : 0;
                const bool withL = h->layersOn || h->bndOn;
                if (withL && h->dMultiIdx && h->dPeer) {
                    hipLaunchKernelGGL(k_halo_combineAL, dim3(nTwo + nMultiBlocks + gridFor(h->nShared)), dim3(kBlock), 0, h->stream, h->nShared, h->dPeer, h->dOwnA,
                                       h->recvA, h->dCombA, nTwo, h->nMulti, h->dMultiIdx, h->dMultiSlots, nTwo + nMultiBlocks, h->st, h->bv, h->bndOn ? 1 : 0,
                                       h->dCombOff, h->dCombSlots, h->dOwnL, h->recvL, h->dCombL, h->dSharedLocal, pushWaitOf(h, 0));
                    return;
                }
                if (nTwo + nMultiBlocks > 0 && h->dMultiIdx && h->dPeer)
                    hipLaunchKernelGGL(k_halo_combineA2, dim3(nTwo + nMultiBlocks), dim3(kBlock), 0, h->stream, h->nShared, h->dPeer, h->dOwnA, h->recvA, h->dCombA,
                                       nTwo, h->nMulti, h->dMultiIdx, h->dMultiSlots, pushWaitOf(h, 0), h->st.ownFold);
                else if (nTwo + nMultiBlocks > 0)
                    hipLaunchKernelGGL(k_halo_combineA, dim3(nTwo + nMultiBlocks), dim3(kBlock), 0, h->stream, h->nShared, h->dCombOff, h->dCombSlots,
                                       h->dOwnA, h->recvA, h->dCombA, &h->st.acc->err, h->dMultiIdx ? 1 : 0, nTwo, h->nMulti, h->dMultiIdx, h->dMultiSlots,
                                       pushWaitOf(h, 0), h->st.ownFold);
                if (withL)
                    hipLaunchKernelGGL(k_halo_combineL, dim3(gridFor(h->nShared)), dim3(kBlock), 0, h->stream, h->nShared, h->dCombOff,
                                       h->dCombSlots, h->dOwnL, h->recvL, h->dCombL, h->st.lStride, h->st.ownFold);
                if (h->bndOn)
                    hipLaunchKernelGGL(k_bnd_normals_shared, dim3(gridFor(h->nShared)), dim3(kBlock), 0, h->stream, h->st, h->bv, h->nShared, h->dSharedLocal);
            })) return 1;
    if (h->useTiles) {
        const int* list = h->interiorDone ? h->dSharedTiles : nullptr;
        const int nList = h->interiorDone ? h->nSharedTiles : 0;
        if (h->interiorDone && nList == 0) {  }
        else if (fused) { if (runSmooth<true>(h, h->mv, h->st, prm, list, nList)) return 1; }
        else if (runSmooth<false>(h, h->mv, h->st, prm, list, nList)) return 1;
        if (h->bndOn) { if (fused ? launchBndFix<true>(h, h->stl.nTiles + gridFor(h->nShared)) : launchBndFix<false>(h, 0)) return 1; }
        if (!fused && runConstraints(h)) return 1;
    } else if (runProposalAndConstraints(h)) return 1;
    if (h->nSend && !(fused && h->st.inlinePackF && !h->bndOn && h->useTiles))
        if (launchK(h, K_HALO, [&] {
                hipLaunchKernelGGL(k_halo_packF, dim3(gridFor(h->nSend)), dim3(kBlock), 0, h->stream, h->nSend, h->dSendShared,
                                   h->dSharedLocal, h->st.frozen, h->sendF, h->st.push, (unsigned)(h->haloIter + 1));
            })) return 1;
    return exchAfterCompute(h);
}

int smgpu_iter_ahead(smgpu_handle* h) {
    if (!h || !h->haloOn) return fail("halo not configured");
    HIP_OK(hipSetDevice(h->device));
    const bool fused = !h->prm.edgeAngleConstraint && !h->prm.faceAngleConstraint;
    if (!h->useTiles || !fused || h->geomAheadDone || !h->useExch || h->mergedIter) return 0;
    if (runGeometry(h, h->dGeomInterior, h->nGeomInterior, true)) return 1;
    h->geomAheadDone = true;
    return 0;
}

int smgpu_iter_end(smgpu_handle* h) {
    if (!h || !h->haloOn) return fail("halo not configured");
    h->iterOpen = false;
    HIP_OK(hipSetDevice(h->device));
    const MeshView& m = h->mv;
    State s = h->st;
    const Prm prm = makePrm(h);
    const bool fused = !h->prm.edgeAngleConstraint && !h->prm.faceAngleConstraint;
    const bool fusedTiles = fused && h->useTiles;
    const bool flg = flagged(h);
    const bool swapHalo = !fusedTiles && s.stepSqr != nullptr;
    if (flg) { if (flagRelay(h, 17, -1)) return 1; }
    else if (computeAfterExch(h)) return 1;
    s.stats = nullptr;
    int nPart;
    if (fusedTiles) {
        const int gS = gridFor(h->nShared);
        if (h->nShared && !(h->mergedIter && h->fixInSmooth))
            if (launchK(h, K_HALO, [&] {
                    hipLaunchKernelGGL(k_shared_fix, dim3(gS), dim3(kBlock), 0, h->stream, m, s, prm, h->nShared, h->dSharedLocal, h->dCombOff,
                                       h->dCombSlots, h->recvF, h->stl.nTiles, pushWaitOf(h, 1), flg ? 1 : 0);
                })) return 1;
        nPart = h->stl.nTiles + (h->bndOn ? gridFor(h->nShared) + gridFor(2 * (int64_t)h->bv.nB) : (h->nShared ? gS : 0));
    } else {
        if (h->nShared && h->nRecv)
            if (launchK(h, K_HALO, [&] {
                    hipLaunchKernelGGL(k_halo_orF, dim3(gridFor(h->nShared)), dim3(kBlock), 0, h->stream, h->nShared, h->dSharedLocal,
                                       h->dCombOff, h->dCombSlots, h->recvF, h->st.frozen, pushWaitOf(h, 1));
                })) return 1;
        if (swapHalo) {
            const int gSwap = (int)((m.nPoints + (int64_t)kApplyPer * kBlock - 1) / ((int64_t)kApplyPer * kBlock));
            if (launchK(h, K_APPLY, [&] { hipLaunchKernelGGL(k_apply_swap, dim3(gSwap), dim3(kBlock), 0, h->stream, m, s, prm); })) return 1;
            nPart = gSwap;
        } else {
            if (launchK(h, K_APPLY, [&] { hipLaunchKernelGGL(k_apply, dim3(gridFor(m.nPoints)), dim3(kBlock), 0, h->stream, m, s, prm); })) return 1;
            nPart = gridFor(m.nPoints);
        }
    }
    double* hist = (h->statsHistory && h->statsHistoryCap > 0) ? h->statsHistory + 2 * (size_t)(h->statsHistoryN++ % h->statsHistoryCap) : nullptr;
    if (hist && (fusedTiles || swapHalo) && h->geomT >= 64 && envInt("SMGPU_DEFER_FINISH", 1)) {
        h->deferN = nPart; h->deferIter = -1 ; h->deferLocal = h->localStats; h->deferHist = hist;
    } else if (launchK(h, K_FINISH, [&] { hipLaunchKernelGGL(k_finish, dim3(1), dim3(kFinishBlock), 0, h->stream, s, nPart, h->haloIter, -1.0, h->localStats, hist); })) return 1;
    if (swapHalo) std::swap(h->st.ptsCur, h->st.prop);
    else std::swap(h->st.ptsCur, h->st.ptsNext);
    if (h->tg.coupled) tangleCoupledIterEnd(h, swapHalo ? h->st.prop : h->st.ptsNext);
    h->haloIter++;
    h->interiorDone = false;
    if (flg && hist) return 0;
    return exchAfterCompute(h);
}

int smgpu_layers_begin(smgpu_handle* h, const smgpu_layer_desc* d, int32_t* enabled, int32_t* maxIter) {
    if (!h || !d) return fail("null argument");
    if (d->nPatches < 0 || (d->nPatches && (!d->patchStart || !d->patchSize || !d->patchKind || !d->isLayerPatch))) return fail("bad patch description");
    HIP_OK(hipSetDevice(h->device));
    bool any = false;
    std::vector<LayerPatch> patches((size_t)d->nPatches);
    for (int i = 0; i < d->nPatches; ++i) {
        patches[(size_t)i] = LayerPatch{d->patchStart[i], d->patchSize[i], (int32_t)d->patchKind[i], d->isLayerPatch[i] != 0};
        any = any || d->isLayerPatch[i];
    }
    const bool on = any && (d->layerMaxBlendingFraction > 1.0e-15);
    if (enabled) *enabled = on ? 1 : 0;
    if (maxIter) *maxIter = d->maxLayers + 1;
    h->layersOn = false;
    h->lb.reset();
    if (!on) return 0;
// ... 611 lines not shown
```

Before: 12.88 billion.

## Streamline tile-kernel prologue with packed launch args, scalar hints and priority boost

Bundles tile-list, meta, stop-word pointer and launch counts into a TileLaunch struct passed as the first kernel argument. The tile id, metadata and stop flag are now fetched at the top of the kernel through constant-address loads, and empty asm constraints pin them in scalar registers. The gather loads for ids, face and cell rows become branch-free with clamped indices. The wave priority is raised during the prologue and dropped before the first barrier. The aim is to shorten the latency-bound kernel start and let index loads issue early, at the cost of extra unconditional loads and possible scalar-register pressure.

Measured after the change: 13.05 billion, median of 6. 1.01x the previous value.

```diff
diff --git a/smoothmesh_amd/csrc/kernels_boundary.hpp b/smoothmesh_amd/csrc/kernels_boundary.hpp
--- a/smoothmesh_amd/csrc/kernels_boundary.hpp
+++ b/smoothmesh_amd/csrc/kernels_boundary.hpp
@@ -152,16 +152,16 @@
 __global__ void __launch_bounds__(64) k_bnd_feature(MeshView m, State s, BndView b) { bndFeatureOf(m, s, b, (int)blockIdx.x, (int)threadIdx.x); }
 
 template <int T, bool ORG>
-__global__ void __launch_bounds__(T, (SMGPU_GEOM_WAVES * T) / 256) k_geom_tile_bnd(MeshView m, State s, GeomTileView g, int wantAvg, int writeFaces,
-                                                  const int* tileList, int nLaunch, int xcdMap, int deferN, int deferIter, double* deferLocal,
-                                                  double* deferHist, BndView b, int nBndBlocks, int nNormalBlocks) {
+__global__ void __launch_bounds__(T, (SMGPU_GEOM_WAVES * T) / 256) k_geom_tile_bnd(TileLaunch tl, MeshView m, State s, GeomTileView g, int wantAvg, int writeFaces,
+                                                  int deferN, int deferIter, double* deferLocal, double* deferHist, BndView b, int nBndBlocks,
+                                                  int nNormalBlocks) {
     const int bx = (int)blockIdx.x;
     if (bx < nBndBlocks) {
         if (bx < nNormalBlocks) bndNormalsOf(m, s, b, bx * T + (int)threadIdx.x);
         else bndFeatureOf(m, s, b, (bx - nNormalBlocks) * (T / 64) + ((int)threadIdx.x >> 6), (int)threadIdx.x & 63);
         return;
     }
-    geomTileBody<T, ORG>(m, s, g, wantAvg, writeFaces, tileList, nLaunch, xcdMap, deferN, deferIter, deferLocal, deferHist, bx - nBndBlocks);
+    geomTileBody<T, ORG>(tl, m, s, g, wantAvg, writeFaces, deferN, deferIter, deferLocal, deferHist, bx - nBndBlocks);
 }
 
 __device__ __forceinline__ bool triangleIntersection(const double* __restrict__ tv, const V3& orig, const V3& dir, double tol, double& t, V3& pt) {
diff --git a/smoothmesh_amd/csrc/kernels_tiled.hpp b/smoothmesh_amd/csrc/kernels_tiled.hpp
--- a/smoothmesh_amd/csrc/kernels_tiled.hpp
+++ b/smoothmesh_amd/csrc/kernels_tiled.hpp
@@ -32,13 +32,14 @@
 struct GeomTileMeta { int tpOff, nPts, tfOff, nFaces, fvBase, fvWidth, cellBeg, nCells, cfBase, cfWidth, flags, pad; };
 constexpr int kGeomMetaInts = 12;
 typedef const __attribute__((address_space(4))) int* const_int_ptr;
-__device__ __forceinline__ GeomTileMeta loadTileMeta(const GeomTileView& g, int tile) {
-    const_int_ptr p = (const_int_ptr)(g.meta + (size_t)kGeomMetaInts * tile);
+__device__ __forceinline__ GeomTileMeta loadGeomMeta(const int* meta, int tile) {
+    const_int_ptr p = (const_int_ptr)(meta + (size_t)kGeomMetaInts * tile);
     GeomTileMeta t;
     t.tpOff = p[0]; t.nPts = p[1]; t.tfOff = p[2]; t.nFaces = p[3]; t.fvBase = p[4]; t.fvWidth = p[5];
     t.cellBeg = p[6]; t.nCells = p[7]; t.cfBase = p[8]; t.cfWidth = p[9]; t.flags = p[10]; t.pad = 0;
     return t;
 }
+__device__ __forceinline__ GeomTileMeta loadTileMeta(const GeomTileView& g, int tile) { return loadGeomMeta(g.meta, tile); }
 
 struct SmoothTileView {
     const int* ptOrder; const int* ptBeg; const int* tcOff; const int* tcIds; const int* tnOff; const int* tnIds;
@@ -63,13 +64,14 @@
 
 struct SmoothTileMeta { int ptBeg, nPts, tcOff, nCells, tnOff, nNbrs, pcBase, pcWidth, ppBase, ppWidth, pfBase, pfWidth; };
 constexpr int kSmoothMetaInts = 12;
-__device__ __forceinline__ SmoothTileMeta loadTileMeta(const SmoothTileView& g, int tile) {
-    const_int_ptr p = (const_int_ptr)(g.meta + (size_t)kSmoothMetaInts * tile);
+__device__ __forceinline__ SmoothTileMeta loadSmoothMeta(const int* meta, int tile) {
+    const_int_ptr p = (const_int_ptr)(meta + (size_t)kSmoothMetaInts * tile);
     SmoothTileMeta t;
     t.ptBeg = p[0]; t.nPts = p[1]; t.tcOff = p[2]; t.nCells = p[3]; t.tnOff = p[4]; t.nNbrs = p[5];
     t.pcBase = p[6]; t.pcWidth = p[7]; t.ppBase = p[8]; t.ppWidth = p[9]; t.pfBase = p[10]; t.pfWidth = p[11];
     return t;
 }
+__device__ __forceinline__ SmoothTileMeta loadTileMeta(const SmoothTileView& g, int tile) { return loadSmoothMeta(g.meta, tile); }
 
 __device__ __forceinline__ int launchTile(int n, int xcdMap, int b = (int)blockIdx.x) {
     if (!xcdMap) return b;
@@ -78,6 +80,32 @@
     return i < n ? i : -1;
 }
 __host__ __device__ inline int tileGrid(int n, int xcdMap) { return xcdMap ? ((n + 7) >> 3) << 3 : n; }
+
+template <class V>
+__device__ __forceinline__ void scalarUse(const V& v) { asm volatile("" : : "s"(v)); }
+template <class... V>
+__device__ __forceinline__ void scalarBatch(const V&... v) { (scalarUse(v), ...); }
+#ifndef SMGPU_PROLOGUE_PRIO
+#define SMGPU_PROLOGUE_PRIO 1
+#endif
+template <int BIT> __device__ __forceinline__ void prologuePrioUp() { if (SMGPU_PROLOGUE_PRIO & BIT) __builtin_amdgcn_s_setprio(2); }
+template <int BIT> __device__ __forceinline__ void prologuePrioDown() { if (SMGPU_PROLOGUE_PRIO & BIT) __builtin_amdgcn_s_setprio(0); }
+struct TileLaunch {
+    const int* meta;
+    const int* tileList;
+    const int* stop;
+    int nLaunch, xcdMap;
+};
+__host__ __device__ inline TileLaunch tileLaunch(const int* meta, const State& s, const int* tileList, int nLaunch, int xcdMap) {
+    return TileLaunch{meta, tileList, reinterpret_cast<const int*>(reinterpret_cast<const char*>(s.acc) + offsetof(Accum, stop)), nLaunch, xcdMap};
+}
+__device__ __forceinline__ int stopWord(const TileLaunch& tl) { return *(const_int_ptr)tl.stop; }
+__device__ __forceinline__ int launchedTile(const TileLaunch& tl, int bid) {
+    scalarBatch(tl.meta, tl.tileList, tl.stop, tl.nLaunch, tl.xcdMap);
+    const int li = launchTile(tl.nLaunch, tl.xcdMap, bid);
+    if (li < 0) return -1;
+    return tl.tileList ? ((const_int_ptr)tl.tileList)[li] : li;
+}
 
 __device__ __forceinline__ V3 ldsv(const double* x, const double* y, const double* z, int i) { return v3(x[i], y[i], z[i]); }
 
@@ -346,17 +374,15 @@
 template <int T>
 __device__ __forceinline__ GeomCellIn geomCellLoad(const GeomTileView& g, const GeomTileMeta& tm, int tid, unsigned tflags) {
     GeomCellIn in;
-    const int ci = tm.cellBeg + tid;
     in.mine = tid < tm.nCells;
-    in.c = 0;
-    in.qa = in.qb = make_ushort4(0, 0, 0, 0);
-    if (in.mine) {
-        in.c = g.cellOrder[ci];
-        if ((tflags & 2u)) {
-            const ushort4* row = reinterpret_cast<const ushort4*>(g.cellFaces + tm.cfBase) + tid;
-            in.qa = row[0]; in.qb = row[T];
-        }
-    }
+    const bool rows = in.mine && (tflags & 2u);
+    const ushort4* cf = reinterpret_cast<const ushort4*>(g.cellFaces);
+    const int r0 = (tm.cfBase >> 2) + tid;
+    const int c = g.cellOrder[in.mine ? tm.cellBeg + tid : 0];
+    const ushort4 qa = cf[rows ? r0 : 0], qb = cf[rows ? r0 + T : 0];
+    const ushort4 zero = make_ushort4(0, 0, 0, 0);
+    in.c = in.mine ? c : 0;
+    in.qa = rows ? qa : zero; in.qb = rows ? qb : zero;
     return in;
 }
 template <int T, bool ORG>
@@ -412,9 +438,12 @@
 #endif
 template <int T>
 __device__ __forceinline__ void geomLoadIds(const GeomTileView& g, const GeomTileMeta& tm, int tid, int (&id)[2]) {
-    const int* ids = g.tpIds + tm.tpOff;
-#pragma unroll
-    for (int u = 0; u < 2; ++u) { const int i = u * T + tid; id[u] = (i < tm.nPts) ? ids[i] : -1; }
+#pragma unroll
+    for (int u = 0; u < 2; ++u) {
+        const int i = u * T + tid;
+        const int v = g.tpIds[(i < tm.nPts) ? tm.tpOff + i : 0];
+        id[u] = (i < tm.nPts) ? v : -1;
+    }
 }
 struct GeomRows { ushort4 fq[2]; GeomCellIn cin; bool preFaces; };
 template <int T, bool ORG>
@@ -425,7 +454,9 @@
 #pragma unroll
     for (int u = 0; u < 2; ++u) {
         const int i = u * T + tid;
-        r.fq[u] = (r.preFaces && i < tm.nFaces) ? reinterpret_cast<const ushort4*>(g.faceVerts + tm.fvBase)[i] : make_ushort4(0, 0, 0, 0);
+        const bool pre = r.preFaces && i < tm.nFaces;
+        const ushort4 q = reinterpret_cast<const ushort4*>(g.faceVerts)[pre ? (tm.fvBase >> 2) + i : 0];
+        r.fq[u] = q;
     }
     r.cin = geomCellLoad<T>(g, tm, tid, tflags);
     return r;
@@ -459,17 +490,18 @@
 }
 
 template <int T, bool ORG>
-__device__ __forceinline__ void geomTileBody(const MeshView& m, const State& s, const GeomTileView& g, int wantAvg, int writeFaces, const int* tileList,
-                                             int nLaunch, int xcdMap, int deferN, int deferIter, double* deferLocal, double* deferHist, int bid, bool coh = false) {
-    const int stopped = s.acc->stop;
-    const int li = launchTile(nLaunch, xcdMap, bid);
-    if (li < 0) return;
+__device__ __forceinline__ void geomTileBody(const TileLaunch& tl, const MeshView& m, const State& s, const GeomTileView& g, int wantAvg, int writeFaces,
+                                             int deferN, int deferIter, double* deferLocal, double* deferHist, int bid, bool coh = false) {
+    const int tile = launchedTile(tl, bid);
+    if (tile < 0) return;
+    const GeomTileMeta tm = loadGeomMeta(tl.meta, tile);
+    const int stopped = stopWord(tl);
+    scalarBatch(tm.tpOff, tm.nPts, tm.tfOff, tm.nFaces, tm.fvBase, tm.fvWidth, tm.cellBeg, tm.nCells, tm.cfBase, tm.cfWidth, tm.flags, stopped,
+                g.tpIds, g.faceVerts, g.cellOrder, g.cellFaces, s.ptsCur, deferN);
     staggerFirstRound(bid, 256 * 4);
     if (deferN > 0 && bid == 0) { if (stopped) return; finishPartials<T>(s, deferN, deferIter, -1.0, deferLocal, deferHist); __syncthreads(); }
     extern __shared__ double lds[];
     const int tid = threadIdx.x;
-    const int tile = tileList ? ((const_int_ptr)tileList)[li] : li;
-    const GeomTileMeta tm = loadTileMeta(g, tile);
     const GeomLds L = geomLds(lds, tm);
     int id[2];
     geomLoadIds<T>(g, tm, tid, id);
@@ -478,6 +510,7 @@
     geomLoadPoints(s, id, v);
     geomStorePoints<T>(s, g, tm, L, id, v, tid);
     if (stopped) return;
+    prologuePrioDown<1>();
     __syncthreads();
     if (SMGPU_ABLATE & 32) { if (tid < tm.nCells) stv(s.cellCtr, ((const_int_ptr)g.cellOrder)[tm.cellBeg + tid], v3(L.px[tid], 0.0, 0.0)); return; }
     geomFaces<T, ORG>(s, g, L, tm, r, tid, wantAvg, writeFaces);
@@ -486,10 +519,10 @@
     geomCell<T, ORG>(s, g, L, tm, tid, (unsigned)tm.flags, r.cin, coh);
 }
 template <int T, bool ORG>
-__global__ void __launch_bounds__(T, (SMGPU_GEOM_WAVES * T) / 256) k_geom_tile(MeshView m, State s, GeomTileView g, int wantAvg, int writeFaces, const int* tileList,
-                                                  int nLaunch, int xcdMap, int deferN, int deferIter, double* deferLocal,
-                                                  double* deferHist) {
-    geomTileBody<T, ORG>(m, s, g, wantAvg, writeFaces, tileList, nLaunch, xcdMap, deferN, deferIter, deferLocal, deferHist, (int)blockIdx.x);
+__global__ void __launch_bounds__(T, (SMGPU_GEOM_WAVES * T) / 256) k_geom_tile(TileLaunch tl, MeshView m, State s, GeomTileView g, int wantAvg, int writeFaces,
+                                                  int deferN, int deferIter, double* deferLocal, double* deferHist) {
+    prologuePrioUp<1>();
+    geomTileBody<T, ORG>(tl, m, s, g, wantAvg, writeFaces, deferN, deferIter, deferLocal, deferHist, (int)blockIdx.x);
 }
 
 struct SmoothLds { double *cx, *cy, *cz, *nx, *ny, *nz; };
@@ -539,6 +572,10 @@
 template <int T, bool COHC = false, int SLOTS = 1>
 __device__ __forceinline__ SmoothRow smoothStage(const MeshView& m, const State& s, const SmoothTileView& g, const SmoothTileMeta& tm,
                                                  const SmoothLds& L, int tid, const SlotTabs& tb = SlotTabs{nullptr, nullptr, nullptr, nullptr}) {
+    scalarBatch(tm.ptBeg, tm.nPts, tm.tcOff, tm.nCells, tm.tnOff, tm.nNbrs, tm.pcBase, tm.pcWidth, tm.ppBase, tm.ppWidth,
+                g.tcIds, g.tnIds, g.ptOrder, g.selfLoc, g.ppEll, g.pcEll, g.pairEll, g.usePairShare, s.cellCtr, s.ptsCur, m.pflags);
+    if (SLOTS == 1) scalarBatch(s.sharedSlot);
+    if (SLOTS == 2) scalarBatch(tb.slot, tb.peer, tb.dst0, tb.ndst);
     SmoothRow r;
     r.peer = -1; r.dst0 = -1; r.ndst = 0;
     r.mine = tid < tm.nPts;
@@ -739,18 +776,20 @@
 }
 
 template <bool FINAL, int T>
-__global__ void __launch_bounds__(T) k_smooth_tile(MeshView m, State s, Prm prm, SmoothTileView g, const int* tileList,
-                                                    int nLaunch, int xcdMap) {
-    const int stopped = s.acc->stop;
-    const int li = launchTile(nLaunch, xcdMap);
-    if (li < 0) return;
+__global__ void __launch_bounds__(T) k_smooth_tile(TileLaunch tl, MeshView m, State s, Prm prm, SmoothTileView g) {
+    prologuePrioUp<2>();
+    const int tile = launchedTile(tl, (int)blockIdx.x);
+    if (tile < 0) return;
+    const SmoothTileMeta tm = loadSmoothMeta(tl.meta, tile);
+    const int stopped = stopWord(tl);
+    scalarBatch(stopped);
     staggerFirstRound((int)blockIdx.x, 256 * 6);
     extern __shared__ double lds[];
-    const int tile = tileList ? ((const_int_ptr)tileList)[li] : li, tid = threadIdx.x;
-    const SmoothTileMeta tm = loadTileMeta(g, tile);
+    const int tid = threadIdx.x;
     const SmoothLds L = smoothLds(lds, tm);
     const SmoothRow R = smoothStage<T>(m, s, g, tm, L, tid);
     if (stopped) return;
+    prologuePrioDown<2>();
     __syncthreads();
     double dist = 0.0;
     int fcount = 0;
@@ -764,13 +803,12 @@
     int centroidAll;
 };
 template <int T, bool COHC = false, bool SP = false>
-__device__ __forceinline__ void packTileBody(const MeshView& m, const State& s, const SmoothTileView& g, const PackView& pk, const int* tileList, int nLaunch,
-                                             int xcdMap, int bid) {
-    const int li = launchTile(nLaunch, xcdMap, bid);
-    if (li < 0) return;
+__device__ __forceinline__ void packTileBody(const TileLaunch& tl, const MeshView& m, const State& s, const SmoothTileView& g, const PackView& pk, int bid) {
+    const int tile = launchedTile(tl, bid);
+    if (tile < 0) return;
     extern __shared__ double lds[];
-    const int tile = tileList ? ((const_int_ptr)tileList)[li] : li, tid = threadIdx.x;
-    const SmoothTileMeta tm = loadTileMeta(g, tile);
+    const int tid = threadIdx.x;
+    const SmoothTileMeta tm = loadSmoothMeta(tl.meta, tile);
     const SmoothLds L = smoothLds(lds, tm);
     const SmoothRow R = smoothStage<T, COHC, SP ? 2 : 1>(m, s, g, tm, L, tid, SlotTabs{s.spSlot, s.spPeer, s.spDst0, s.spNDst});
     __syncthreads();
@@ -840,11 +878,10 @@
     }
 }
 template <int T>
-__global__ void __launch_bounds__(T) k_pack_tile(MeshView m, State s, SmoothTileView g, PackView pk, const int* tileList, int nLaunch,
-                                                  int xcdMap, PackLArgs la, int nLBlocks, unsigned tag) {
-    if (s.acc->stop) return;
+__global__ void __launch_bounds__(T) k_pack_tile(TileLaunch tl, MeshView m, State s, SmoothTileView g, PackView pk, PackLArgs la, int nLBlocks, unsigned tag) {
+    if (stopWord(tl)) return;
     if ((int)blockIdx.x < nLBlocks) haloPackLOf(s, la, (int)blockIdx.x * T + (int)threadIdx.x);
-    else packTileBody<T>(m, s, g, pk, tileList, nLaunch, xcdMap, (int)blockIdx.x - nLBlocks);
+    else packTileBody<T>(tl, m, s, g, pk, (int)blockIdx.x - nLBlocks);
     pushSignal(s.push, 0, tag);
 }
 
@@ -857,14 +894,15 @@
     int debug;
 };
 template <int T, bool ORG>
-__global__ void __launch_bounds__(T, (SMGPU_GEOM_WAVES * T) / 256) k_geom_halo(MeshView m, State s, GeomTileView g, int writeFaces, HaloG hg, int xcdMap, int deferN,
+__global__ void __launch_bounds__(T, (SMGPU_GEOM_WAVES * T) / 256) k_geom_halo(TileLaunch tl, MeshView m, State s, GeomTileView g, int writeFaces, HaloG hg, int deferN,
                                                                               int deferIter, double* deferLocal, double* deferHist, SmoothTileView sg, PackView pk) {
+    const int xcdMap = tl.xcdMap;
     const int bid = (int)blockIdx.x, gS = tileGrid(hg.nGeomS, xcdMap), g1 = tileGrid(hg.nI1, xcdMap), gP = tileGrid(hg.nPack, xcdMap);
     if (bid >= gS + g1 && bid < gS + g1 + gP) {
-        if (s.acc->stop || (hg.debug & 1)) return;
+        if (stopWord(tl) || (hg.debug & 1)) return;
         __builtin_amdgcn_s_setprio(3);
         if (!(hg.debug & 2)) roleWait(hg.ticket, hg.serial, &s.acc->err);
-        packTileBody<T, true, true>(m, s, sg, pk, nullptr, hg.nPack, xcdMap, bid - gS - g1);
+        packTileBody<T, true, true>(TileLaunch{sg.meta, nullptr, tl.stop, hg.nPack, xcdMap}, m, s, sg, pk, bid - gS - g1);
         pushSignal(s.push, 0, hg.tagA, (unsigned)gP);
         return;
     }
@@ -872,7 +910,7 @@
     const int* list = first ? hg.geomS : (second ? hg.geomI : hg.geomI + hg.nI1);
     const int n = first ? hg.nGeomS : (second ? hg.nI1 : hg.nGeomI - hg.nI1);
     const int b = first ? bid : (second ? bid - gS : bid - gS - g1 - gP);
-    geomTileBody<T, ORG>(m, s, g, 0, writeFaces, list, n, xcdMap, first ? deferN : 0, deferIter, deferLocal, deferHist, b, first);
+    geomTileBody<T, ORG>(TileLaunch{tl.meta, list, tl.stop, n, xcdMap}, m, s, g, 0, writeFaces, first ? deferN : 0, deferIter, deferLocal, deferHist, b, first);
     if (first) roleDone(hg.ticket, hg.serial, (unsigned)gS >> 3);
 }
 
@@ -917,8 +955,8 @@
     blockPublish<T>(s, dist, fcount, hf.partialBase + blk);
 }
 template <int T>
-__global__ void __launch_bounds__(T) k_smooth_halo(MeshView m, State s, Prm prm, SmoothTileView g, SmoothTileView sg, HaloS hs, int xcdMap, HaloFix hf) {
-    const int bid = (int)blockIdx.x, tid = threadIdx.x;
+__global__ void __launch_bounds__(T) k_smooth_halo(TileLaunch tl, MeshView m, State s, Prm prm, SmoothTileView g, SmoothTileView sg, HaloS hs, HaloFix hf) {
+    const int bid = (int)blockIdx.x, tid = threadIdx.x, xcdMap = tl.xcdMap;
     if (bid < hs.gM) {
         if (bid >= hs.nMultiBlocks) return;
         __builtin_amdgcn_s_setprio(3);
@@ -944,7 +982,7 @@
     if (li < 0 && !spTile) return;
     if (!spTile && !batchA) li += hs.nA;
     const int tile = li >= 0 ? li : 0;
-    const SmoothTileMeta tm = loadTileMeta(v, tile);
+    const SmoothTileMeta tm = loadSmoothMeta(spTile ? sg.meta : tl.meta, tile);
     const SmoothLds L = smoothLds(lds, tm);
     if (spTile) {
         const int pi = tm.ptBeg + ((tid < tm.nPts) ? tid : 0);
diff --git a/smoothmesh_amd/csrc/quality_loop.hpp b/smoothmesh_amd/csrc/quality_loop.hpp
--- a/smoothmesh_amd/csrc/quality_loop.hpp
+++ b/smoothmesh_amd/csrc/quality_loop.hpp
@@ -40,8 +40,8 @@
                                        h->xcdMap, h->qt.thr, h->qt.cellPart, gate);
                 } else {
                     ensureDynLds(k_geom_tile<T, ORG>, h->device, h->geomLds);
-                    hipLaunchKernelGGL((k_geom_tile<T, ORG>), dim3(tileGrid(nT, h->xcdMap)), dim3(T), (uint32_t)h->geomLds, h->stream, h->mv, ts, h->gv, 0, 1,
-                                       (const int*)nullptr, nT, h->xcdMap, 0, 0, (double*)nullptr, (double*)nullptr);
+                    hipLaunchKernelGGL((k_geom_tile<T, ORG>), dim3(tileGrid(nT, h->xcdMap)), dim3(T), (uint32_t)h->geomLds, h->stream,
+                                       tileLaunch(h->gv.meta, ts, nullptr, nT, h->xcdMap), h->mv, ts, h->gv, 0, 1, 0, 0, (double*)nullptr, (double*)nullptr);
                 }
             });
     } else {
diff --git a/smoothmesh_amd/csrc/smgpu.hip b/smoothmesh_amd/csrc/smgpu.hip
--- a/smoothmesh_amd/csrc/smgpu.hip
+++ b/smoothmesh_amd/csrc/smgpu.hip
@@ -1206,8 +1206,8 @@
 template <bool FINAL, int T>
 static void launchSmoothTile(smgpu_handle* h, const MeshView& m, const State& s, const Prm& prm, const int* tileList, int nTiles, hipEvent_t evA, hipEvent_t evB) {
     ensureDynLds(k_smooth_tile<FINAL, T>, h->device, h->smoothLds);
-    hipExtLaunchKernelGGL((k_smooth_tile<FINAL, T>), dim3(tileGrid(nTiles, h->xcdMap)), dim3(T), (uint32_t)h->smoothLds, h->stream, evA, evB, 0, m, s, prm, h->sv,
-                          tileList, nTiles, h->xcdMap);
+    hipExtLaunchKernelGGL((k_smooth_tile<FINAL, T>), dim3(tileGrid(nTiles, h->xcdMap)), dim3(T), (uint32_t)h->smoothLds, h->stream, evA, evB, 0,
+                          tileLaunch(h->sv.meta, s, tileList, nTiles, h->xcdMap), m, s, prm, h->sv);
 }
 template <bool FINAL>
 static int launchBndFix(smgpu_handle* h, int partialBase) {
@@ -1279,13 +1279,14 @@
                     const int nNormal = (h->bv.nB + T - 1) / T, nFeat = (h->bv.nFeat + (T / 64) - 1) / (T / 64);
                     const int nBnd = ((nNormal + nFeat + 7) / 8) * 8;
                     ensureDynLds(k_geom_tile_bnd<T, ORG>, h->device, h->geomLds);
-                    hipExtLaunchKernelGGL((k_geom_tile_bnd<T, ORG>), dim3(nBnd + tileGrid(nT, h->xcdMap)), dim3(T), (uint32_t)h->geomLds, h->stream, evA, evB, 0, m, s,
-                                          h->gv, wantAvg, h->writeFaces ? 1 : 0, tileList, nT, h->xcdMap, h->deferN, h->deferIter, h->deferLocal, h->deferHist, h->bv,
-                                          nBnd, nNormal);
+                    hipExtLaunchKernelGGL((k_geom_tile_bnd<T, ORG>), dim3(nBnd + tileGrid(nT, h->xcdMap)), dim3(T), (uint32_t)h->geomLds, h->stream, evA, evB, 0,
+                                          tileLaunch(h->gv.meta, s, tileList, nT, h->xcdMap), m, s, h->gv, wantAvg, h->writeFaces ? 1 : 0, h->deferN, h->deferIter,
+                                          h->deferLocal, h->deferHist, h->bv, nBnd, nNormal);
                 } else {
                     ensureDynLds(k_geom_tile<T, ORG>, h->device, h->geomLds);
-                    hipExtLaunchKernelGGL((k_geom_tile<T, ORG>), dim3(tileGrid(nT, h->xcdMap)), dim3(T), (uint32_t)h->geomLds, h->stream, evA, evB, 0, m, s, h->gv,
-                                          wantAvg, h->writeFaces ? 1 : 0, tileList, nT, h->xcdMap, h->deferN, h->deferIter, h->deferLocal, h->deferHist);
+                    hipExtLaunchKernelGGL((k_geom_tile<T, ORG>), dim3(tileGrid(nT, h->xcdMap)), dim3(T), (uint32_t)h->geomLds, h->stream, evA, evB, 0,
+                                          tileLaunch(h->gv.meta, s, tileList, nT, h->xcdMap), m, s, h->gv, wantAvg, h->writeFaces ? 1 : 0, h->deferN, h->deferIter,
+                                          h->deferLocal, h->deferHist);
                 }
             });
             h->deferN = 0;
@@ -2424,13 +2425,14 @@
     hg.debug = envInt("SMGPU_HALO_DEBUG", 0);
     const PackView pk{h->dOwnA, h->sendA, h->dSendOff, h->dSendSlots, 0};
     const size_t lds = std::max(h->geomLds, h->haloLds);
+    const TileLaunch tl = tileLaunch(h->gv.meta, s, nullptr, 0, h->xcdMap);
     const int rc = launchKDispatch(h, K_GEOM_TILE, [&](hipEvent_t evA, hipEvent_t evB) {
         if (h->foamOrg)
-            hipExtLaunchKernelGGL((k_geom_halo<256, true>), dim3(gS + g1 + gP + g2), dim3(256), (uint32_t)lds, h->stream, evA, evB, 0, m, s, h->gv, h->writeFaces ? 1 : 0, hg,
-                                  h->xcdMap, h->deferN, h->deferIter, h->deferLocal, h->deferHist, h->hv, pk);
+            hipExtLaunchKernelGGL((k_geom_halo<256, true>), dim3(gS + g1 + gP + g2), dim3(256), (uint32_t)lds, h->stream, evA, evB, 0, tl, m, s, h->gv,
+                                  h->writeFaces ? 1 : 0, hg, h->deferN, h->deferIter, h->deferLocal, h->deferHist, h->hv, pk);
         else
-            hipExtLaunchKernelGGL((k_geom_halo<256, false>), dim3(gS + g1 + gP + g2), dim3(256), (uint32_t)lds, h->stream, evA, evB, 0, m, s, h->gv, h->writeFaces ? 1 : 0, hg,
-                                  h->xcdMap, h->deferN, h->deferIter, h->deferLocal, h->deferHist, h->hv, pk);
+            hipExtLaunchKernelGGL((k_geom_halo<256, false>), dim3(gS + g1 + gP + g2), dim3(256), (uint32_t)lds, h->stream, evA, evB, 0, tl, m, s, h->gv,
+                                  h->writeFaces ? 1 : 0, hg, h->deferN, h->deferIter, h->deferLocal, h->deferHist, h->hv, pk);
     });
     h->deferN = 0;
     h->deferLocal = h->deferHist = nullptr;
@@ -2464,7 +2466,8 @@
     if (flagged(h)) s.push = h->flagView;
     s.ownF = h->fixInSmooth ? h->dOwnF : nullptr;
     return launchKDispatch(h, K_SMOOTH_FINAL, [&](hipEvent_t evA, hipEvent_t evB) {
-        hipExtLaunchKernelGGL((k_smooth_halo<256>), dim3(grid), dim3(256), (uint32_t)lds, h->stream, evA, evB, 0, h->mv, s, prm, h->sv, h->hv, hs, h->xcdMap, hf);
+        hipExtLaunchKernelGGL((k_smooth_halo<256>), dim3(grid), dim3(256), (uint32_t)lds, h->stream, evA, evB, 0,
+                              tileLaunch(h->sv.meta, s, nullptr, 0, h->xcdMap), h->mv, s, prm, h->sv, h->hv, hs, hf);
     });
 }
 
@@ -2516,9 +2519,10 @@
                     const PackView pk{h->dOwnA, h->sendA, h->dSendOff, h->dSendSlots, h->bndOn ? 1 : 0};
                     const int T = h->smoothT, nL = withL ? (((h->nShared + T - 1) / T + 7) / 8) * 8 : 0;
                     const dim3 grid(nL + tileGrid(h->nSharedTiles, h->xcdMap));
-                    if (T == 64) hipLaunchKernelGGL(k_pack_tile<64>, grid, dim3(64), h->smoothLds, h->stream, m, s, h->sv, pk, h->dSharedTiles, h->nSharedTiles, h->xcdMap, la, nL, tag);
-                    else if (T == 128) hipLaunchKernelGGL(k_pack_tile<128>, grid, dim3(128), h->smoothLds, h->stream, m, s, h->sv, pk, h->dSharedTiles, h->nSharedTiles, h->xcdMap, la, nL, tag);
-                    else hipLaunchKernelGGL(k_pack_tile<256>, grid, dim3(256), h->smoothLds, h->stream, m, s, h->sv, pk, h->dSharedTiles, h->nSharedTiles, h->xcdMap, la, nL, tag);
+                    const TileLaunch tl = tileLaunch(h->sv.meta, s, h->dSharedTiles, h->nSharedTiles, h->xcdMap);
+                    if (T == 64) hipLaunchKernelGGL(k_pack_tile<64>, grid, dim3(64), h->smoothLds, h->stream, tl, m, s, h->sv, pk, la, nL, tag);
+                    else if (T == 128) hipLaunchKernelGGL(k_pack_tile<128>, grid, dim3(128), h->smoothLds, h->stream, tl, m, s, h->sv, pk, la, nL, tag);
+                    else hipLaunchKernelGGL(k_pack_tile<256>, grid, dim3(256), h->smoothLds, h->stream, tl, m, s, h->sv, pk, la, nL, tag);
                 } else {
                     hipLaunchKernelGGL(k_halo_packA, dim3(gridFor(h->nShared)), dim3(kBlock), 0, h->stream, m, s, h->dSharedLocal, h->dOwnA, h->nShared,
                                        h->dSendOff, h->dSendSlots, h->sendA, h->bndOn ? 1 : 0);
```
